# cucapra/pollen

Hardware: AMD Instinct MI355X
Metric: path-steps/sec on `depth` (1M seg / 100M step GFA); bit-exact vs flatgfa CPU (higher is better)
Workload: dtype u32

## Files before the change

pollen_amd/csrc/depth_accum.hip:

```cpp
#include <hip/hip_runtime.h>

#include <cstdlib>

#include "depth_fast_kernels.hpp"
#include "depth_sorted_host.hpp"

namespace fgfa_dev {
namespace {


template <bool UNIQ, int WB>
__device__ __forceinline__ void apply_record(int *D, int *R, uint32_t rec) {
    constexpr uint32_t kW = 1u << WB;
    const uint32_t rel = rec & (kW - 1), end = rel + ((rec >> WB) & ((1u << (kTagShift - WB)) - 1u)) + 1;
    if (UNIQ) {
        const int d = (int)((rec >> 24) & 1u), rv = d - (int)((rec >> 25) & 1u);
        if (d) {
            atomicAdd(&D[rel], 1);
            atomicAdd(&D[end], -1);
        }
        if (rv) {
            atomicAdd(&R[rel], rv);
            atomicAdd(&R[end], -rv);
        }
    } else {
        atomicAdd(&D[rel], 1);
        atomicAdd(&D[end], -1);
    }
}

constexpr uint32_t kPend = 96;
constexpr uint32_t kPendRun = 32;
struct Pending {
    uint32_t *m;
    uint2 *r;
    uint32_t mcnt, rcnt;
    uint32_t moldest;
    int lane;
};

__device__ __forceinline__ uint32_t claim_word(uint32_t *bits, bool act, uint32_t &p, uint32_t e, uint32_t &base) {
    uint32_t rv = 0;
    base = p & ~31u;
    if (act) {
        const uint32_t lo = p & 31u, wl = min(e, p | 31u), width = wl - p + 1u;
        const uint32_t mask = (0xFFFFFFFFu >> (32u - width)) << lo;
        rv = mask & atomicOr(&bits[p >> 5], mask);
        p = wl + 1u;
    }
    return rv;
}
__device__ __forceinline__ void park_rest(Pending &q, bool e, uint32_t val) {
    const unsigned long long mk = __builtin_amdgcn_ballot_w64(e);
    if (e) q.m[q.mcnt + lane_rank(mk)] = val;
    q.mcnt = __builtin_amdgcn_readfirstlane(q.mcnt + (uint32_t)__builtin_popcountll(mk));
}
__device__ __forceinline__ void park_revisit(Pending &q, bool e, uint32_t base, uint32_t rv) {
    const unsigned long long mk = __builtin_amdgcn_ballot_w64(e);
    if (e) q.r[q.rcnt + lane_rank(mk)] = make_uint2(base, rv);
    q.rcnt = __builtin_amdgcn_readfirstlane(q.rcnt + (uint32_t)__builtin_popcountll(mk));
}
template <int WB, int PB = 13>
__device__ __forceinline__ void run_rest(Pending &q, uint32_t *mybits, uint32_t dbg) {
    constexpr uint32_t kNW = (1u << WB) / 32u, kPM = (1u << PB) - 1u;
    const uint32_t n = __builtin_amdgcn_readfirstlane(min(q.mcnt, 64u));
    q.mcnt = __builtin_amdgcn_readfirstlane(q.mcnt - n);
    const bool act = (uint32_t)q.lane < n;
    const uint32_t v = act ? q.m[q.mcnt + q.lane] : 0u;
    asm volatile("" ::: "memory");
    uint32_t p = v & kPM, base;
    const uint32_t e = (v >> PB) & kPM;
    uint32_t rv = claim_word(mybits + (v >> (2 * PB)) * kNW, act, p, e, base);
    if (dbg & kDbgNoRevisit) rv = 0;
    park_rest(q, act && p <= e, (v & ~kPM) | p);
    park_revisit(q, rv != 0u, base, rv);
}
__device__ __forceinline__ void run_revisits(Pending &q, int *R) {
    const uint32_t n = __builtin_amdgcn_readfirstlane(min(q.rcnt, 64u));
    q.rcnt = __builtin_amdgcn_readfirstlane(q.rcnt - n);
    const bool act = (uint32_t)q.lane < n;
    const uint2 v = act ? q.r[q.rcnt + q.lane] : make_uint2(0u, 0u);
    asm volatile("" ::: "memory");
    uint32_t rv = v.y;
    if (rv) {
        const uint32_t low = rv & (0u - rv), sum = rv + low;
        const uint32_t from = (uint32_t)__builtin_ctz(low), to = sum ? (uint32_t)__builtin_ctz(sum) : 32u;
        rv &= sum;
        atomicAdd(&R[v.x + from], 1);
        atomicAdd(&R[v.x + to], -1);
    }
    park_revisit(q, rv != 0u, v.x, rv);
}
template <int WB, int PB = 13>
__device__ __forceinline__ void run_pending(Pending &q, int *R, uint32_t *mybits, uint32_t dbg, uint32_t at_least) {
    while (q.mcnt >= at_least || q.rcnt >= at_least) {
        if (q.rcnt >= at_least) run_revisits(q, R);
        else run_rest<WB, PB>(q, mybits, dbg);
        if (at_least == 1u && q.mcnt == 0u && q.rcnt == 0u) break;
    }
}

struct Claim {
    uint32_t old, mask, p, e, base, slot;
    bool act;
};
template <int WB, bool POINT = false>
__device__ __forceinline__ Claim claim_begin(int *D, Pending &q, uint32_t *mybits, uint32_t slot, uint32_t hfirst, uint32_t rec, bool valid, uint32_t dbg) {
    constexpr uint32_t kW = 1u << WB, kNW = kW / 32u;
    Claim c;
    const uint32_t rel = rec & (kW - 1);
    if (POINT) {
        c.e = rel;
        if (valid) {
            atomicAdd(&D[rel], 1);
            atomicAdd(&D[rel + 1u], -1);
        }
        c.act = valid;
        c.slot = slot;
        c.base = rel & ~31u;
        c.mask = 1u << (rel & 31u);
        c.p = rel + 1u;
        c.old = valid ? atomicOr(&mybits[slot * kNW + (rel >> 5)], c.mask) : 0u;
        return c;
    }
    c.e = rel + ((rec >> WB) & 1023u);
    if (valid && !(dbg & kDbgNoDepth)) {
        atomicAdd(&D[rel], 1);
        atomicAdd(&D[c.e + 1u], -1);
    }
    c.act = valid && !(dbg & kDbgNoClaim);
    c.slot = slot;
    c.base = rel & ~31u;
    const uint32_t lo = rel & 31u, wl = min(c.e, rel | 31u), width = wl - rel + 1u;
    c.mask = (0xFFFFFFFFu >> (32u - width)) << lo;
    c.p = wl + 1u;
    c.old = c.act ? atomicOr(&mybits[slot * kNW + (rel >> 5)], c.mask) : 0u;
    if (q.mcnt == 0u) q.moldest = __builtin_amdgcn_readfirstlane(hfirst);
    return c;
}
template <int WB, bool POINT = false, int PB = 13>
__device__ __forceinline__ void claim_end(int *R, Pending &q, uint32_t *mybits, const Claim &c, uint32_t dbg) {
    uint32_t rv = c.act ? (c.mask & c.old) : 0u;
    if (dbg & kDbgNoRevisit) rv = 0;
    if (POINT) {
        if (rv) {
            atomicAdd(&R[c.e], 1);
            atomicAdd(&R[c.e + 1u], -1);
        }
        return;
    }
    park_rest(q, c.act && c.p <= c.e, c.p | (c.e << PB) | (c.slot << (2 * PB)));
    park_revisit(q, rv != 0u, c.base, rv);
    run_pending<WB, PB>(q, R, mybits, dbg, kPendRun);
}

template <typename T, int N>
__device__ __forceinline__ void block_scan(T *wave_tot, T (&v)[N]) {
    const int tid = threadIdx.x, lane = tid & 63, wave = tid >> 6;
#pragma unroll
    for (int k = 1; k < N; ++k) v[k] += v[k - 1];
    T incl = v[N - 1];
    for (int off = 1; off < 64; off <<= 1) {
        const T t = __shfl_up(incl, off, 64);
        if (lane >= off) incl += t;
    }
    if (lane == 63) wave_tot[wave] = incl;
    __syncthreads();
    T add = incl - v[N - 1];
    for (int k = 0; k < wave; ++k) add += wave_tot[k];
    __syncthreads();
#pragma unroll
    for (int k = 0; k < N; ++k) v[k] += add;
}

template <int N>
__device__ __forceinline__ void store_n(uint32_t *out, uint32_t i0, uint32_t nvalid, const uint32_t (&a)[N]) {
    if (N == 2) {
        if (i0 + 1 < nvalid) *reinterpret_cast<uint2 *>(out + i0) = make_uint2(a[0], a[1]);
        else if (i0 < nvalid) out[i0] = a[0];
        return;
    }
#pragma unroll
    for (int k0 = 0; k0 + 3 < N; k0 += 4) {
        if (i0 + k0 + 3 < nvalid) {
            *reinterpret_cast<uint4 *>(out + i0 + k0) = make_uint4(a[k0], a[k0 + 1], a[k0 + 2], a[k0 + 3]);
        } else {
            for (uint32_t k = 0; k < 4; ++k)
                if (i0 + k0 + k < nvalid) out[i0 + k0 + k] = a[k0 + k];
        }
    }
}

template <int N>
__device__ __forceinline__ void add_n(uint32_t *out, uint32_t i0, uint32_t nvalid, const uint32_t (&a)[N]) {
#pragma unroll
    for (int k = 0; k < N; ++k)
        if (a[k] && i0 + k < nvalid) atomicAdd(out + i0 + k, a[k]);
}

template <bool UNIQ, int kPer>
__device__ __forceinline__ void window_counts(const int *D, const int *R, unsigned long long *wave_tot, uint32_t i0, uint32_t (&d)[kPer], uint32_t (&rv)[kPer]) {
    if (UNIQ) {
        unsigned long long v[kPer];
#pragma unroll
        for (int k = 0; k < kPer; ++k) v[k] = (unsigned long long)(long long)D[i0 + k] + ((unsigned long long)(long long)R[i0 + k] << 32);
        block_scan<unsigned long long, kPer>(wave_tot, v);
#pragma unroll
        for (int k = 0; k < kPer; ++k) {
            d[k] = (uint32_t)v[k];
            rv[k] = (uint32_t)(v[k] >> 32);
        }
    } else {
        int v[kPer];
#pragma unroll
        for (int k = 0; k < kPer; ++k) v[k] = D[i0 + k];
        block_scan<int, kPer>(reinterpret_cast<int *>(wave_tot), v);
#pragma unroll
        for (int k = 0; k < kPer; ++k) d[k] = (uint32_t)v[k];
    }
}
template <bool UNIQ, int kPer>
__device__ __forceinline__ void write_counts(const AccArgs &A, uint32_t w0, uint32_t i0, uint32_t nvalid, bool add, const uint32_t (&d)[kPer], const uint32_t (&u)[kPer]) {
    if (add) {
        add_n<kPer>(A.depth_out + w0, i0, nvalid, d);
        if (UNIQ) add_n<kPer>(A.uniq_out + w0, i0, nvalid, u);
    } else {
        store_n<kPer>(A.depth_out + w0, i0, nvalid, d);
        if (UNIQ) store_n<kPer>(A.uniq_out + w0, i0, nvalid, u);
    }
}

template <bool UNIQ, int WB, int kPerRound = 16>
__device__ __forceinline__ void apply_flat(const AccArgs &A, int *D, int *R, const uint32_t *scnt, const uint32_t *sstart, const uint32_t *wbase) {
    const int lane = threadIdx.x & 63;
    const uint32_t uw = __builtin_amdgcn_readfirstlane(blockIdx.y * kAccWaves + (threadIdx.x >> 6)), nw = A.parts * kAccWaves;
    for (uint32_t s0 = uw; s0 < A.n_slots; s0 += kPerRound * nw) {
        uint4 r[kPerRound];
        uint32_t cnt[kPerRound];
#pragma unroll
        for (int k = 0; k < kPerRound; ++k) {
            const uint32_t s = s0 + k * nw;
            const uint32_t sc = s < A.n_slots ? s : 0u;
            cnt[k] = s < A.n_slots ? scnt[sc] : 0u;
            r[k] = reinterpret_cast<const uint4 *>(wbase + sstart[sc])[(uint32_t)lane < (cnt[k] >> 2) ? lane : 0];
        }
#pragma unroll
        for (int k = 0; k < kPerRound; ++k) {
            if ((uint32_t)lane < (cnt[k] >> 2)) {
                apply_record<UNIQ, WB>(D, R, r[k].x);
                apply_record<UNIQ, WB>(D, R, r[k].y);
                apply_record<UNIQ, WB>(D, R, r[k].z);
                apply_record<UNIQ, WB>(D, R, r[k].w);
            }
        }
#pragma unroll 1
        for (int k = 0; k < kPerRound; ++k) {
            const uint32_t s = s0 + k * nw;
            if (s >= A.n_slots) break;
            const uint32_t c = scnt[s];
            const uint32_t *bk = wbase + sstart[s];
            for (uint32_t i = 64 + lane; i < (c >> 2); i += 64) {
                const uint4 v = reinterpret_cast<const uint4 *>(bk)[i];
                apply_record<UNIQ, WB>(D, R, v.x);
                apply_record<UNIQ, WB>(D, R, v.y);
                apply_record<UNIQ, WB>(D, R, v.z);
                apply_record<UNIQ, WB>(D, R, v.w);
            }
            const uint32_t rest = (c & ~3u) + lane;
            if (rest < c) apply_record<UNIQ, WB>(D, R, bk[rest]);
        }
    }
}

template <int K>
__device__ __forceinline__ void rec_request(const uint32_t *p) {
#ifndef FGFA_REC_POLICY
#define FGFA_REC_POLICY ""
#endif
    if (K == 0) asm volatile("global_load_dword v120, %0, off" FGFA_REC_POLICY ::"v"(p) : "memory", "v120");
    else if (K == 1) asm volatile("global_load_dword v121, %0, off" FGFA_REC_POLICY ::"v"(p) : "memory", "v121");
    else asm volatile("global_load_dword v122, %0, off" FGFA_REC_POLICY ::"v"(p) : "memory", "v122");
}
template <int K>
__device__ __forceinline__ uint32_t rec_take() {
    uint32_t r;
    if (K == 0) asm volatile("s_waitcnt vmcnt(2)\n\tv_mov_b32 %0, v120" : "=v"(r)::"memory");
    else if (K == 1) asm volatile("s_waitcnt vmcnt(2)\n\tv_mov_b32 %0, v121" : "=v"(r)::"memory");
    else asm volatile("s_waitcnt vmcnt(2)\n\tv_mov_b32 %0, v122" : "=v"(r)::"memory");
    return r;
}

template <int WB, bool SHARED, bool POINT, bool BIG>
__device__ __forceinline__ void apply_groups(const AccArgs &A, int *D, int *R, uint32_t *mybits, uint32_t *mark, uint32_t *pend, const uint32_t *wbase, uint32_t win,
                                             uint32_t e0, uint32_t e1, bool have_first = false, uint2 be_first = make_uint2(0u, 0u), uint32_t slf_first = 0u) {
    constexpr uint32_t kNW = (1u << WB) / 32u;
    constexpr uint32_t kSlots = WB <= 12 ? 8u : 4u;
    const int lane = threadIdx.x & 63;
    const uint32_t wave = __builtin_amdgcn_readfirstlane(blockIdx.y * kAccWaves + (threadIdx.x >> 6)), nw = A.parts * kAccWaves;
    const uint32_t nback = (A.has_pre && !SHARED) ? min(__builtin_amdgcn_readfirstlane(*A.work_counter), A.max_back) : 0u;
    const uint32_t nst = e1 - e0;
    const uint32_t nE = nst + (nback > wave ? (nback - wave + nw - 1u) / nw : 0u);
    uint32_t gbase = 0, carryG = 0;
    uint32_t hbase = 0, hdone = 0;
    Pending pq;
    pq.m = pend;
    pq.r = reinterpret_cast<uint2 *>(pend + kPend);
    pq.mcnt = pq.rcnt = pq.moldest = 0;
    pq.lane = lane;
    uint2 be_next = make_uint2(0u, 0u);
    uint32_t slf_next = 0u;
    const auto fetch = [&](uint32_t mb) {
        const uint32_t x = mb + (uint32_t)lane;
        const uint32_t at = x < nst ? e0 + x : A.n_items + wave + nw * (x - nst);
        be_next = x < nE ? A.dir[(size_t)win * A.dstride + at] : make_uint2(0u, 0u);
        slf_next = x < nE ? A.islot[at] : 0u;
    };
    if (have_first) {
        be_next = be_first;
        slf_next = slf_first;
    } else {
        fetch(0);
    }
    for (uint32_t mb = 0; mb < nE; mb += 64u) {
        const uint2 be = be_next;
        const uint32_t slf = slf_next;
        fetch(mb + 64u);
        const uint32_t sl = slf & 0x7FFFFFFFu, first = slf >> 31;
        const uint32_t b = min(be.x, A.cap), en = max(b, min(be.y, A.cap));
        const uint32_t n = en - b;
        const uint32_t incl = wave_scan_incl(n), P = incl - n;
        const uint32_t T = __builtin_amdgcn_readlane(incl, 63);
        const uint32_t G = gbase + wave_scan_incl(first);
        gbase = __builtin_amdgcn_readlane(G, 63);
        const unsigned long long ne = __builtin_amdgcn_ballot_w64(n != 0u);
        const unsigned long long below = ne & ((1ull << lane) - 1ull);
        const int pv = below ? 63 - __builtin_clzll(below) : 0;
        const uint32_t gsh = __shfl(G, pv, 64);
        const uint32_t gprev = below ? gsh : carryG;
        const uint32_t H = hbase + wave_scan_incl((n != 0u && gprev != G) ? 1u : 0u);
        hbase = __builtin_amdgcn_readlane(H, 63);
        if (ne) carryG = __builtin_amdgcn_readlane(G, 63 - __builtin_clzll(ne));
        const uint32_t offH = (sl * A.cap + b) | (H << 24);
        uint32_t cs = 0, lastE = 0;
        uint32_t curEnd = 0;
        uint32_t hseen = hdone;
        struct Chunk {
            const uint32_t *src;
            uint32_t slot;
            uint32_t nv, hl, hf;
        };
        auto prep = [&]() -> Chunk {
            Chunk c;
            const uint32_t q = cs + (uint32_t)lane;
            if (BIG && cs + 64u <= curEnd) {
                const uint32_t oh = __builtin_amdgcn_readlane(offH, lastE), Ps = __builtin_amdgcn_readlane(P, lastE);
                const uint32_t h = oh >> 24;
                c.hf = c.hl = h;
                c.nv = 64u;
                c.src = wbase + (oh & 0xFFFFFFu) + (q - Ps);
                c.slot = h & (kSlots - 1u);
                hseen = h;
                cs += 64u;
                return c;
            }
            const uint32_t relp = P - cs;
            mark[lane] = 0u;
            if (n != 0u && relp < 64u) mark[relp] = (uint32_t)lane + 1u;
            asm volatile("" ::: "memory");
            const uint32_t sel = max(wave_scan_max(mark[lane]), lastE + 1u) - 1u;
            const uint32_t oh = __shfl(offH, (int)sel, 64), Ps = __shfl(P, (int)sel, 64);
            const uint32_t h = oh >> 24;
// ... 626 lines not shown
        const uint32_t at = x < nst ? ge0 + x : A.n_items + vwave + nw * (x - nst);
        if (x < nE) {
            be_first = A.dir[(size_t)win * A.dstride + at];
            slf_first = A.islot[at];
        }
    }
    for (uint32_t sl = tid; sl < A.n_slots; sl += kAccThreads) {
        if ((sl % nw) / kAccWaves != blockIdx.y) {
            sstart[sl] = A.pk ? A.pk[(size_t)win * A.n_slots + sl].x : sl * A.cap;
            continue;
        }
        uint32_t *c = A.counts + (size_t)win * A.n_slots + sl;
        uint32_t v = *c;
        if (!A.keep) *c = 0u;
        uint32_t start = sl * A.cap, room = A.cap;
        if (A.pk) {
            const uint2 e = A.pk[(size_t)win * A.n_slots + sl];
            start = e.x;
            room = e.y;
        } else if (v > (A.cap >> 1)) {
            atomicMax(A.status + 2, v);
            if (A.fullest) atomicMax(A.fullest, v);
        }
        sstart[sl] = start;
        if (TAGGED && UNIQ) {
            const uint32_t c1 = min(v, room);
            v = min(A.has_pre == 1 ? A.counts0[(size_t)win * A.n_slots + sl] : A.has_pre ? v : 0u, c1);
            scnt2[sl] = make_uint2(start + v, (c1 - v) | (A.taken && A.taken[sl] <= (uint32_t)SLOTS ? 0x80000000u : 0u));
        } else if (UNIQ && A.has_pre == 1) {
            v = A.counts0[(size_t)win * A.n_slots + sl];
        }
        scnt[sl] = min(v, room);
    }
    if (tid == 0) grab = kAccWaves;
    if (TAGGED && UNIQ)
        for (uint32_t i = tid; i < A.n_shared * (kW / 32); i += kAccThreads) tag_bits[kAccWaves * (uint32_t)SLOTS * (kW / 32) + i] = 0u;
    const uint32_t nvalid = min(kW, A.n_segs - w0);
    for (uint32_t i = tid; i < (UNIQ ? 2u : 1u) * (kW + 64); i += kAccThreads) cells[i] = 0;
    __syncthreads();
    const uint32_t *wbase = A.pk ? A.buckets : A.buckets + (size_t)win * A.n_slots * A.cap;
    tm.mark(0);
    if (flat) apply_flat<UNIQ, WB, (LOWREG ? 4 : 16)>(A, D, R, scnt, sstart, wbase);
    tm.mark(1);
    if (UNIQ && TAGGED) {
        if (PAIR) apply_tagged<WB, POINT, false, true, (int)kTagSlots, NC>(A, D, R, tag_bits, scnt2, wbase, &grab);
        else if (LOWREG && A.n_shared) apply_tagged<WB, POINT, true, true, SLOTS, NC>(A, D, R, tag_bits, scnt2, wbase, &grab);
        else if (LOWREG) apply_tagged<WB, POINT, false, true, SLOTS, NC>(A, D, R, tag_bits, scnt2, wbase, &grab);
        else if (A.n_shared) apply_tagged<WB, POINT, true, false, SLOTS, NC, OWN>(A, D, R, tag_bits, scnt2, wbase, &grab);
        else apply_tagged<WB, POINT, false, false, SLOTS, NC, OWN>(A, D, R, tag_bits, scnt2, wbase, &grab);
    } else if (UNIQ) {
        apply_groups<WB, false, POINT, BIG>(A, D, R, bits + wave * (kSlots * (kW / 32)), marks + wave * 64, pend + wave * (3 * kPend), wbase, win,
                                ge0, ge1, true, be_first, slf_first);
        for (uint32_t f = A.fat_off[blockIdx.y]; f < A.fat_off[blockIdx.y + 1]; ++f) {
            __syncthreads();
            for (uint32_t i = tid; i < kW / 32; i += kAccThreads) bits[kW / 32 + i] = 0u;
            __syncthreads();
            const uint32_t *wo = A.fat_woff + (size_t)f * (kAccWaves + 1) + wave;
            apply_groups<WB, true, POINT, BIG>(A, D, R, bits, marks + wave * 64, pend + wave * (3 * kPend), wbase, win,
                                   __builtin_amdgcn_readfirstlane(wo[0]), __builtin_amdgcn_readfirstlane(wo[1]));
        }
    }
    tm.mark(2);
    __syncthreads();
    tm.mark(3);
    const uint32_t i0 = kPer * tid;
    uint32_t d[kPer], u[kPer];
    if (UNIQ) {
        uint32_t rv[kPer];
        window_counts<true, kPer>(D, R, wave_tot, i0, d, rv);
#pragma unroll
        for (int k = 0; k < kPer; ++k) u[k] = d[k] - rv[k];
        if (PAIR) {
            __shared__ uint32_t second;
            uint32_t *mine = A.pair_part + ((size_t)win * 2u + blockIdx.y) * (2u * kW);
            const uint32_t *theirs = A.pair_part + ((size_t)win * 2u + (1u - blockIdx.y)) * (2u * kW);
#pragma unroll
            for (int k = 0; k < kPer; ++k) {
                __hip_atomic_store(mine + i0 + k, d[k], __ATOMIC_RELAXED, __HIP_MEMORY_SCOPE_AGENT);
                __hip_atomic_store(mine + kW + i0 + k, rv[k], __ATOMIC_RELAXED, __HIP_MEMORY_SCOPE_AGENT);
            }
            asm volatile("s_waitcnt vmcnt(0)" ::: "memory");
            __syncthreads();
            if (tid == 0) second = __hip_atomic_fetch_add(&A.pair_flag[win], 1u, __ATOMIC_RELAXED, __HIP_MEMORY_SCOPE_AGENT);
            __syncthreads();
            if (second) {
#pragma unroll
                for (int k = 0; k < kPer; ++k) {
                    d[k] += __hip_atomic_load(theirs + i0 + k, __ATOMIC_RELAXED, __HIP_MEMORY_SCOPE_AGENT);
                    rv[k] += __hip_atomic_load(theirs + kW + i0 + k, __ATOMIC_RELAXED, __HIP_MEMORY_SCOPE_AGENT);
                }
#pragma unroll
                for (int k = 0; k < kPer; ++k) u[k] = d[k] - rv[k];
                if (A.accumulate) {
                    add_n<kPer>(A.depth_out + w0, i0, nvalid, d);
                    add_n<kPer>(A.uniq_out + w0, i0, nvalid, u);
                } else {
                    store_n<kPer>(A.depth_out + w0, i0, nvalid, d);
                    store_n<kPer>(A.uniq_out + w0, i0, nvalid, u);
                }
                if (tid == 0) __hip_atomic_store(&A.pair_flag[win], 0u, __ATOMIC_RELAXED, __HIP_MEMORY_SCOPE_AGENT);
            }
        } else {
            write_counts<true, kPer>(A, w0, i0, nvalid, A.parts > 1 || A.accumulate, d, u);
        }
        tm.mark(4);
        tm.finish();
    } else {
        window_counts<false, kPer>(D, R, wave_tot, i0, d, u);
        write_counts<false, kPer>(A, w0, i0, nvalid, !PSUM && (A.parts > 1 || A.accumulate), d, u);
        if (PSUM) {
            unsigned long long l[kPer], w[kPer];
#pragma unroll
            for (int k = 0; k < kPer; ++k) {
                const uint32_t len = i0 + k < nvalid ? A.seg_len[w0 + i0 + k] : 0u;
                l[k] = len;
                w[k] = (unsigned long long)d[k] * len;
            }
            block_scan<unsigned long long, kPer>(wave_tot, l);
            block_scan<unsigned long long, kPer>(wave_tot, w);
#pragma unroll
            for (int k = 0; k < kPer; ++k) {
                LW[i0 + k + 1] = make_ulonglong2(l[k], w[k]);
            }
            if (tid == 0) LW[0] = make_ulonglong2(0ull, 0ull);
            __syncthreads();
            sum_groups<WB>(A, LW, wbase, win, __builtin_amdgcn_readfirstlane(A.wave_off[vwave]), __builtin_amdgcn_readfirstlane(A.wave_off[vwave + 1]));
            for (uint32_t f = A.fat_off[blockIdx.y]; f < A.fat_off[blockIdx.y + 1]; ++f) {
                const uint32_t *wo = A.fat_woff + (size_t)f * (kAccWaves + 1) + wave;
                sum_groups<WB>(A, LW, wbase, win, __builtin_amdgcn_readfirstlane(wo[0]), __builtin_amdgcn_readfirstlane(wo[1]));
            }
        }
    }
}

template <bool UNIQ, int WB, bool PSUM = false, bool POINT = false, bool BIG = false, bool TAGGED = false, int SLOTS = (int)kTagSlots, bool NC = false, bool OWN = false>
__global__ __launch_bounds__(kAccThreads) void k_accum(const AccArgs A) {
    accum_body<UNIQ, WB, PSUM, POINT, BIG, TAGGED, false, SLOTS, false, NC, OWN>(A);
}
#ifdef FGFA_MEASURE
template <int WB, bool POINT>
__global__ __launch_bounds__(kAccThreads) __attribute__((amdgpu_waves_per_eu(8, 8))) void k_accum_pair(const AccArgs A) {
    accum_body<true, WB, false, POINT, false, true, true, (int)kTagSlots, true, true>(A);
}
template <int WB>
__global__ __launch_bounds__(kAccThreads) __attribute__((amdgpu_waves_per_eu(8, 8))) void k_accum_small(const AccArgs A) {
    accum_body<true, WB, false, false, false, true, false, (int)kTagSlots, true, true>(A);
}
#endif

typedef uint32_t sorted_u32x4 __attribute__((ext_vector_type(4)));
template <bool NT>
__device__ __forceinline__ sorted_u32x4 sorted_load4(const sorted_u32x4 *p) { return NT ? __builtin_nontemporal_load(p) : *p; }

template <bool UNIQ, int WB, bool CHECKED>
__device__ __forceinline__ void sweep_group(int *D, int *R, const sorted_u32x4 &r4, uint32_t carry, bool in, int lane) {
    const uint32_t pad = CHECKED && !in ? kSortedPad : 0u;
    const uint32_t rec[kSortedGroup] = {r4.x | pad, r4.y | pad, r4.z | pad, r4.w | pad};
    if (UNIQ) {
        const uint32_t q = (uint32_t)lane >> 4, seed = CHECKED && !in ? 0u : sorted_seed(q, carry);
        SortedLane ln;
        sorted_lane_keys<CHECKED>(rec, q, (uint32_t)WB, seed, ln);
        uint32_t p = sorted_umax(seed, wave_scan_max((uint32_t)__builtin_amdgcn_update_dpp(0u, ln.t, 0x138 , 0xf, 0xf, true)));
#pragma unroll
        for (uint32_t k = 0; k < kSortedGroup; ++k) {
            uint32_t end;
            const bool hit = sorted_record_step<CHECKED>(p, ln.x[k], ln.len[k], end);
            if (!CHECKED || ln.x[k] != 0u) {
                atomicAdd(&D[ln.s[k]], 1);
                atomicAdd(&D[ln.s[k] + ln.len[k] + 1u], -1);
            }
            if (hit) {
                atomicAdd(&R[ln.s[k]], 1);
                atomicAdd(&R[end], -1);
            }
        }
    } else {
        constexpr uint32_t kW = 1u << WB;
#pragma unroll
        for (uint32_t k = 0; k < kSortedGroup; ++k) {
            const uint32_t s = rec[k] & (kW - 1u), e = s + ((rec[k] >> WB) & 1023u) + 1u;
            if (!CHECKED || !(rec[k] & kSortedPad)) {
                atomicAdd(&D[s], 1);
                atomicAdd(&D[e], -1);
            }
        }
    }
}

template <bool UNIQ, int WB, bool NT>
__global__ __launch_bounds__(kAccThreads) __attribute__((amdgpu_waves_per_eu(8, 8))) void k_accum_sorted(const AccArgs A) {
    static_assert(kSortedChunk == 64u && kSortedGroup == 4u, "a lane holds four consecutive records of one chunk: sixteen lanes a chunk");
    constexpr uint32_t kW = 1u << WB;
    constexpr int kPer = kW / kAccThreads;
    __shared__ __attribute__((aligned(16))) int cells[(UNIQ ? 2 : 1) * (kW + 64)];
    __shared__ unsigned long long wave_tot[kAccWaves];
    int *D = cells, *R = cells + (UNIQ ? kW + 64 : 0);
    const int tid = threadIdx.x, lane = tid & 63;
    const uint32_t wave = __builtin_amdgcn_readfirstlane(tid >> 6);
    const uint32_t win = blockIdx.x, w0 = win * kW;
    const uint32_t c0 = __builtin_amdgcn_readfirstlane(A.swin_chunk[win]), c1 = __builtin_amdgcn_readfirstlane(A.swin_chunk[win + 1]);
    const uint32_t ng = (c1 - c0 + kSortedGroup - 1u) / kSortedGroup;
    const sorted_u32x4 *img = reinterpret_cast<const sorted_u32x4 *>(A.srec);
    const uint32_t q = (uint32_t)lane >> 4;
    uint32_t g = wave;
    sorted_u32x4 ra, rb;
    uint32_t ca = 0u, cb = 0u;
    const auto request = [&](sorted_u32x4 &r, uint32_t &cy, uint32_t at) {
        const uint32_t ck = c0 + at * kSortedGroup;
        r = sorted_load4<NT>(img + min(ck * (kSortedChunk / kSortedGroup) + (uint32_t)lane, c1 * (kSortedChunk / kSortedGroup) - 1u));
        if (UNIQ) cy = A.scarry[min(ck + q, c1 - 1u)];
    };
    const auto sweep = [&](const sorted_u32x4 &r, uint32_t cy, uint32_t at) {
        if (at + 1u == ng) sweep_group<UNIQ, WB, true>(D, R, r, cy, c0 + at * kSortedGroup + q < c1, lane);
        else sweep_group<UNIQ, WB, false>(D, R, r, cy, true, lane);
    };
    if (ng) request(ra, ca, g);
    for (uint32_t i = tid; i < (UNIQ ? 2u : 1u) * (kW + 64); i += kAccThreads) cells[i] = 0;
    __syncthreads();
    while (g < ng) {
        request(rb, cb, g + kAccWaves);
        sweep(ra, ca, g);
        g += kAccWaves;
        if (g >= ng) break;
        request(ra, ca, g + kAccWaves);
        sweep(rb, cb, g);
        g += kAccWaves;
    }
    __syncthreads();
    const uint32_t nvalid = min(kW, A.n_segs - w0), i0 = kPer * tid;
    uint32_t d[kPer], u[kPer];
    window_counts<UNIQ, kPer>(D, R, wave_tot, i0, d, u);
    if (UNIQ) {
#pragma unroll
        for (int k = 0; k < kPer; ++k) u[k] = d[k] - u[k];
    }
    write_counts<UNIQ, kPer>(A, w0, i0, nvalid, A.accumulate != 0u, d, u);
}

}

bool accum_kernels_setup() {
    static OncePerDevice once;
    const bool ok = once([] {
        bool good = true;
        const auto set = [&](const void *k, uint32_t bytes) { good = hipFuncSetAttribute(k, hipFuncAttributeMaxDynamicSharedMemorySize, (int)bytes) == hipSuccess && good; };
        set((const void *)k_accum<true, 11, false, false, false, true>, tagged_lds_bytes(11, kMaxShared));
        set((const void *)k_accum<true, 12, false, false, false, true>, tagged_lds_bytes(12, kMaxShared));
        set((const void *)k_accum<true, 12, false, true, false, true>, tagged_lds_bytes(12, kMaxShared));
        set((const void *)k_accum<true, 12, false, false, false, true, 8>, tagged_lds_bytes(12, 64, 8));
        set((const void *)k_accum<true, 13, false, false, false, true>, tagged_lds_bytes(13, 0));
        set((const void *)k_accum<true, 13, false, true, false, true>, tagged_lds_bytes(13, 0));
        set((const void *)k_accum<true, 11, false, false, false, true, (int)kTagSlots, true>, tagged_lds_bytes(11, kMaxShared));
        set((const void *)k_accum<true, 12, false, false, false, true, (int)kTagSlots, true>, tagged_lds_bytes(12, kMaxShared));
        set((const void *)k_accum<true, 12, false, true, false, true, (int)kTagSlots, true>, tagged_lds_bytes(12, kMaxShared));
        set((const void *)k_accum<true, 12, false, false, false, true, 8, true>, tagged_lds_bytes(12, 64, 8));
        set((const void *)k_accum<true, 13, false, false, false, true, (int)kTagSlots, true>, tagged_lds_bytes(13, 0));
        set((const void *)k_accum<true, 13, false, true, false, true, (int)kTagSlots, true>, tagged_lds_bytes(13, 0));
        set((const void *)k_accum<true, 12, false, false, false, true, (int)kTagSlots, false, true>, tagged_lds_bytes(12, kMaxShared));
        set((const void *)k_accum<true, 12, false, false, false, true, 8, false, true>, tagged_lds_bytes(12, 64, 8));
        set((const void *)k_accum<true, 13, false, false, false, true, (int)kTagSlots, false, true>, tagged_lds_bytes(13, 0));
        set((const void *)k_accum<true, 12, false, false, false, true, (int)kTagSlots, true, true>, tagged_lds_bytes(12, kMaxShared));
        set((const void *)k_accum<true, 12, false, false, false, true, 8, true, true>, tagged_lds_bytes(12, 64, 8));
        set((const void *)k_accum<true, 13, false, false, false, true, (int)kTagSlots, true, true>, tagged_lds_bytes(13, 0));
#ifdef FGFA_MEASURE
        set((const void *)k_accum_small<11>, tagged_lds_bytes(11, kMaxShared));
        set((const void *)k_accum_pair<12, false>, tagged_lds_bytes(12, 0));
        set((const void *)k_accum_pair<12, true>, tagged_lds_bytes(12, 0));
#endif
        return good;
    });
    if (!ok) set_error("hipFuncSetAttribute(k_accum): dynamic shared memory");
    return ok;
}

#define FGFA_TAGGED_LAUNCH(GRID, LDS, WB_, POINT_, SLOTS_)                                                                      \
    do {                                                                                                                       \
        if (nc) hipLaunchKernelGGL((k_accum<true, WB_, false, POINT_, false, true, SLOTS_, true>), GRID, dim3(kAccThreads), LDS, stream, aa);  \
        else hipLaunchKernelGGL((k_accum<true, WB_, false, POINT_, false, true, SLOTS_, false>), GRID, dim3(kAccThreads), LDS, stream, aa);    \
    } while (0)
#define FGFA_OWN_LAUNCH(GRID, LDS, WB_, SLOTS_)                                                                                \
    do {                                                                                                                       \
        if (nc) hipLaunchKernelGGL((k_accum<true, WB_, false, false, false, true, SLOTS_, true, true>), GRID, dim3(kAccThreads), LDS, stream, aa);  \
        else hipLaunchKernelGGL((k_accum<true, WB_, false, false, false, true, SLOTS_, false, true>), GRID, dim3(kAccThreads), LDS, stream, aa);    \
    } while (0)
#define FGFA_SORTED_LAUNCH(WB_)                                                                                                  \
    do {                                                                                                                        \
        if (uniq && fp.sorted_nt) hipLaunchKernelGGL((k_accum_sorted<true, WB_, true>), dim3(fp.n_win), dim3(kAccThreads), 0, stream, aa);        \
        else if (uniq) hipLaunchKernelGGL((k_accum_sorted<true, WB_, false>), dim3(fp.n_win), dim3(kAccThreads), 0, stream, aa);                  \
        else if (fp.sorted_nt) hipLaunchKernelGGL((k_accum_sorted<false, WB_, true>), dim3(fp.n_win), dim3(kAccThreads), 0, stream, aa);          \
        else hipLaunchKernelGGL((k_accum_sorted<false, WB_, false>), dim3(fp.n_win), dim3(kAccThreads), 0, stream, aa);                           \
    } while (0)
void launch_accum(const FastPlan &fp, AccArgs &aa, bool uniq, bool tagged, bool psum, hipStream_t stream, bool sorted) {
    if (sorted) {
        if (fp.wb == 11) FGFA_SORTED_LAUNCH(11);
        else if (fp.wb == 12) FGFA_SORTED_LAUNCH(12);
        else FGFA_SORTED_LAUNCH(13);
        return;
    }
    const dim3 agrid(fp.n_win, fp.acc_parts);
    const bool pair = uniq && tagged && fp.acc_pair;
    const bool nc = fp.n_noclaim != 0 || fp.n_flag_chunks != 0;
#ifdef FGFA_MEASURE
    if (pair) {
        aa.parts = 2;
        const uint32_t tl = tagged_lds_bytes(fp.wb, 0);
        const dim3 pgrid(fp.n_win, 2);
        if (fp.dense) hipLaunchKernelGGL((k_accum_pair<12, true>), pgrid, dim3(kAccThreads), tl, stream, aa);
        else hipLaunchKernelGGL((k_accum_pair<12, false>), pgrid, dim3(kAccThreads), tl, stream, aa);
    } else
#else
    (void)pair;
#endif
    if (uniq && tagged) {
        const uint32_t tl = tagged_lds_bytes(fp.wb, fp.n_shared);
        if (fp.dense && fp.wb == 12) FGFA_TAGGED_LAUNCH(agrid, tl, 12, true, (int)kTagSlots);
        else if (fp.dense && fp.wb == 13) FGFA_TAGGED_LAUNCH(agrid, tl, 13, true, (int)kTagSlots);
#ifdef FGFA_MEASURE
        else if (fp.wb == 11 && test_hook("FLATGFA_ACC_SMALL")) hipLaunchKernelGGL((k_accum_small<11>), agrid, dim3(kAccThreads), tl, stream, aa);
#endif
        else if (fp.wb == 11) FGFA_TAGGED_LAUNCH(agrid, tl, 11, false, (int)kTagSlots);
        else if (fp.acc_own && fp.wb == 12 && fp.acc_slots == 8 && fp.n_shared <= 64) FGFA_OWN_LAUNCH(agrid, tagged_lds_bytes(12, fp.n_shared, 8), 12, 8);
        else if (fp.acc_own && fp.wb == 12) FGFA_OWN_LAUNCH(agrid, tl, 12, (int)kTagSlots);
        else if (fp.acc_own && fp.wb == 13) FGFA_OWN_LAUNCH(agrid, tl, 13, (int)kTagSlots);
        else if (fp.wb == 12 && fp.acc_slots == 8 && fp.n_shared <= 64) FGFA_TAGGED_LAUNCH(agrid, tagged_lds_bytes(12, fp.n_shared, 8), 12, false, 8);
        else if (fp.wb == 12) FGFA_TAGGED_LAUNCH(agrid, tl, 12, false, (int)kTagSlots);
        else FGFA_TAGGED_LAUNCH(agrid, tl, 13, false, (int)kTagSlots);
    } else if (uniq) {
        const bool big = fp.big_groups;
        if (fp.dense && fp.wb == 12 && big) hipLaunchKernelGGL((k_accum<true, 12, false, true, true>), agrid, dim3(kAccThreads), 0, stream, aa);
        else if (fp.dense && fp.wb == 12) hipLaunchKernelGGL((k_accum<true, 12, false, true, false>), agrid, dim3(kAccThreads), 0, stream, aa);
        else if (fp.dense && fp.wb == 13) hipLaunchKernelGGL((k_accum<true, 13, false, true, true>), agrid, dim3(kAccThreads), 0, stream, aa);
        else if (fp.wb == 12 && big) hipLaunchKernelGGL((k_accum<true, 12, false, false, true>), agrid, dim3(kAccThreads), 0, stream, aa);
        else if (fp.wb == 13 && big) hipLaunchKernelGGL((k_accum<true, 13, false, false, true>), agrid, dim3(kAccThreads), 0, stream, aa);
        else if (fp.wb == 11) hipLaunchKernelGGL((k_accum<true, 11>), agrid, dim3(kAccThreads), 0, stream, aa);
        else if (fp.wb == 12) hipLaunchKernelGGL((k_accum<true, 12>), agrid, dim3(kAccThreads), 0, stream, aa);
        else hipLaunchKernelGGL((k_accum<true, 13>), agrid, dim3(kAccThreads), 0, stream, aa);
    } else {
        if (fp.wb == 11) hipLaunchKernelGGL((k_accum<false, 11>), agrid, dim3(kAccThreads), 0, stream, aa);
        else if (fp.wb == 12 && psum) hipLaunchKernelGGL((k_accum<false, 12, true>), agrid, dim3(kAccThreads), 0, stream, aa);
        else if (fp.wb == 12) hipLaunchKernelGGL((k_accum<false, 12>), agrid, dim3(kAccThreads), 0, stream, aa);
        else hipLaunchKernelGGL((k_accum<false, 13>), agrid, dim3(kAccThreads), 0, stream, aa);
    }
}
#undef FGFA_TAGGED_LAUNCH
#undef FGFA_OWN_LAUNCH
#undef FGFA_SORTED_LAUNCH

void launch_path_reduce(const FastPlan &fp, unsigned long long *len_out, unsigned long long *weighted_out, hipStream_t stream) {
    hipLaunchKernelGGL(k_path_reduce, dim3((fp.n_items + 3) / 4), dim3(256), 0, stream, reinterpret_cast<const uint4 *>(fp.items), fp.elist, fp.n_items,
                       fp.n_win, fp.dstride, reinterpret_cast<const ulonglong2 *>(fp.psum_part), len_out, weighted_out);
}

}
```

pollen_amd/csrc/depth_call_host.hpp:

```cpp
#pragma once
#include <algorithm>
#include <cstdint>

#include "depth_fast.hpp"

namespace fgfa_dev {

struct CallHooks {
    bool scan_always = false;
    const char *scan_time = nullptr;
    bool no_plain = false;
    bool acc_time = false;
    const char *acc_skip = nullptr;
};
struct CallWants {
    bool uniq = false;
    bool psum = false, psum_clear = false;
    bool count_only = false;
};
struct GraphFacts {
    uint32_t n_segs;
    bool has_seg_len;
};
enum class Zeroes { nobody, k_scan, memset };
struct CallShape {
    const char *refusal = nullptr;
    bool has_pre = false;
    bool scan_skip = false;
    uint32_t grid = 0;
    uint32_t grid_tiny = 0, grid_short = 0, grid_medium = 0;
    bool tagged = false, ranged = false, big = false, cflags = false;
    bool from_image = false;
    bool kept = false;
    bool sorted = false;
    uint32_t has_pre2 = 0;
    uint32_t max_back = 0;
    Zeroes outputs = Zeroes::nobody, sums = Zeroes::nobody;
    bool scans() const { return grid && !kept; }
};

constexpr int kModeDense = -1, kModeRefused = -2;
struct ScanMode {
    int mode;
    bool tagged;
};
inline ScanMode scan_mode(const FastPlan &fp, const CallShape &s) {
    if (fp.dense) return {kModeDense, false};
#ifdef FGFA_MEASURE
    if (fp.dbg) return {kModeDbg, false};
#endif
    const bool flags = s.cflags && s.tagged && !s.ranged;
    if (flags && fp.packed) return {kModePackedFlags, true};
    if (flags && !s.big) return {kModePlainFlags, true};
    if (fp.packed) return {s.ranged ? kModePackedRanged : kModePacked, true};
    if (s.big && !s.tagged) return {kModeRefused, false};
    if (s.big) return {s.ranged ? kModeRangedBig : kModeBig, true};
    if (s.ranged) return {kModeRanged, s.tagged};
    return {s.tagged && fp.narrow_emit ? kModePlainNarrow : kModePlain, s.tagged};
}

inline uint32_t wave_list_grid(uint32_t n, uint32_t per_wg, uint32_t n_slots) { return std::min<uint32_t>((n + per_wg - 1) / per_wg, n_slots); }

inline CallShape decide_call(const FastPlan &fp, const GraphFacts &g, const CallWants &w, const CallHooks &hooks, bool records_use) {
    CallShape s;
    if (w.psum && (w.uniq || fp.wb != 12 || !g.has_seg_len || !fp.psum_part || fp.n_range != g.n_segs)) {
        s.refusal = "fast_seg_depth: path sums ride on seg_depth with 4096-segment windows only";
        return s;
    }
    const bool tagged = fp.tagged && !w.psum;
    if (fp.packed && !tagged) {
        s.refusal = "fast_seg_depth: a plan with packed buckets runs tagged calls only";
        return s;
    }
    s.tagged = tagged;
    s.has_pre = fp.n_short || fp.n_medium || fp.n_tiny;
    s.scan_skip = s.has_pre && fp.n_items == 0 && fp.exact_short && !fp.dbg && !hooks.scan_always;
    s.grid = s.scan_skip ? 0u : s.has_pre ? fp.n_slots : std::min<uint32_t>(fp.n_items, fp.n_slots);
    s.has_pre2 = s.scan_skip ? 2u : s.has_pre ? 1u : 0u;
    s.max_back = s.scan_skip ? 0u : fp.max_back;
    s.ranged = fp.seg_base != 0 || fp.n_range != g.n_segs;
    const uint32_t stride = fp.n_slots * fp.cap;
    s.big = ((uint64_t)fp.n_win + 1) * stride >= (1ull << 30);
    s.cflags = tagged && fp.cflags;
    s.from_image = s.grid && tagged && fp.run_ent && fp.run_item_ent && !w.count_only && !fp.dense && !fp.packed && !s.ranged && !s.cflags && !s.has_pre && !fp.dbg;
    s.kept = s.from_image && records_use && fp.counts_kept;
    s.sorted = s.kept && fp.sorted_rec && fp.sorted_carry && fp.sorted_win_chunk && fp.acc_parts == 1 && fp.wb >= 11 && fp.wb <= 13;
    if (s.scans() && !s.from_image && scan_mode(fp, s).mode == kModeRefused) {
        CallShape no;
        no.refusal = "fast_seg_depth: a bucket array this large needs a tagged call";
        return no;
    }
    if (fp.n_tiny) s.grid_tiny = wave_list_grid(fp.n_tiny, kWaves, fp.n_slots);
    if (fp.n_short) s.grid_short = wave_list_grid(fp.n_short, kShortWaves, fp.n_slots);
    if (fp.n_medium) s.grid_medium = wave_list_grid(fp.n_medium, kMediumPaired ? kMediumWaves / 2 : kMediumWaves, fp.n_slots);
    const Zeroes who = s.scans() ? Zeroes::k_scan : Zeroes::memset;
    if (fp.acc_parts > 1 && !fp.accumulate && !w.count_only) s.outputs = who;
    if (w.psum && w.psum_clear) s.sums = s.grid ? Zeroes::k_scan : Zeroes::memset;
    return s;
}

enum class StatusVerdict {
    fine,
    bounds, stale, internal, several_calls,
    redo_grown,
    redo_atomic,
    unresolved,
};
struct StatusAction {
    StatusVerdict verdict;
    bool grow_ahead;
};
inline StatusAction status_verdict(const uint32_t st3[3], uint32_t calls, int attempt, bool last_fast, bool has_last_call) {
    const uint32_t st = st3[0], over = kStOverflow | kStBackOverflow;
    StatusAction a{StatusVerdict::fine, st3[2] != 0 && !(st & over)};
    if (st & kStBounds) a.verdict = StatusVerdict::bounds;
    else if (st & kStStale) a.verdict = StatusVerdict::stale;
    else if (st & kStInternal) a.verdict = StatusVerdict::internal;
    else if (!(st & over)) a.verdict = StatusVerdict::fine;
    else if (attempt == 0 && calls > 1) a.verdict = StatusVerdict::several_calls;
    else if (!last_fast || !has_last_call || attempt > 8) a.verdict = StatusVerdict::unresolved;
    else a.verdict = (st & kStBackOverflow) ? StatusVerdict::redo_atomic : StatusVerdict::redo_grown;
    return a;
}

}
```

pollen_amd/csrc/depth_device.hip:

```cpp
#include <hip/hip_runtime.h>

#include <algorithm>
#include <atomic>
#include <chrono>
#include <cstdio>
#include <cstdlib>
#include <cstring>
#include <mutex>
#include <string>
#include <vector>

#include "../../include/flatgfa.h"
#include "depth_call_host.hpp"
#include "depth_fast.hpp"
#include "depth_sorted_host.hpp"
#include "temp_arena.hpp"
#include "host_copy.hpp"
#include "device_common.hpp"
#include "prof.hpp"

namespace fgfa_dev {

thread_local std::string g_last_error;
void set_error(const std::string &s) { g_last_error = s; }
// ... 91 lines not shown
            if (seg >= n_segs) {
                *status = 1u;
                continue;
            }
            if (win == 0) atomicAdd(&depth[seg], 1u);
            const uint32_t rel = seg - lo;
            if (rel < nbits) {
                const uint32_t bit = 1u << (rel & 31u);
                const uint32_t old = atomicOr(&seen[rel >> 5], bit);
                if (!(old & bit)) atomicAdd(&uniq[seg], 1u);
            }
        }
        __syncthreads();
    }
}

constexpr int kSumThreads = 256;

__global__ __launch_bounds__(256) void k_zero_outputs(uint32_t *__restrict__ a, uint32_t *__restrict__ b, uint32_t n) {
    for (uint32_t i = blockIdx.x * 256u + threadIdx.x; i < n; i += gridDim.x * 256u) {
        a[i] = 0u;
        if (b) b[i] = 0u;
    }
}

__global__ __launch_bounds__(256) void k_pack_len_depth(const uint32_t *__restrict__ seg_len,
                                                        const uint32_t *__restrict__ depth, uint32_t n_segs,
                                                        uint2 *__restrict__ tab) {
    for (uint32_t s = blockIdx.x * blockDim.x + threadIdx.x; s < n_segs; s += gridDim.x * blockDim.x)
        tab[s] = make_uint2(seg_len[s], depth[s]);
}

__global__ __launch_bounds__(kSumThreads) void k_path_sums(const uint32_t *__restrict__ steps,
                                                            const uint32_t *__restrict__ path_begin,
                                                            const uint32_t *__restrict__ path_end, uint32_t n_paths,
                                                            uint32_t n_segs, const uint2 *__restrict__ tab,
                                                            const uint32_t *__restrict__ path_ids, uint32_t n_ids,
                                                            uint32_t split, uint32_t by_path,
                                                            unsigned long long *__restrict__ length_out,
                                                            unsigned long long *__restrict__ weighted_out,
                                                            uint32_t *__restrict__ status) {
    __shared__ unsigned long long red[2][kSumThreads / 64];
    const uint64_t total = (uint64_t)n_ids * split;
    for (uint64_t job = blockIdx.x; job < total; job += gridDim.x) {
        const uint32_t k = (uint32_t)(job / split), part = (uint32_t)(job % split);
        const uint32_t p = path_ids[k];
        unsigned long long len = 0, wsum = 0;
        if (p < n_paths) {
            const uint64_t b = path_begin[p], e = path_end[p];
            const uint64_t n = e - b;
            const uint64_t lo = b + n * part / split, hi = b + n * (part + 1) / split;
            constexpr int kBatch = 8;
            bool bad = false;
            uint64_t i = lo + threadIdx.x;
            for (; i + (uint64_t)(kBatch - 1) * kSumThreads < hi; i += (uint64_t)kBatch * kSumThreads) {
                uint32_t seg[kBatch];
                uint2 ld[kBatch];
#pragma unroll
                for (int k = 0; k < kBatch; ++k) seg[k] = steps[i + (uint64_t)k * kSumThreads] >> 1;
#pragma unroll
                for (int k = 0; k < kBatch; ++k) {
                    bad |= seg[k] >= n_segs;
                    ld[k] = tab[seg[k] < n_segs ? seg[k] : 0u];
                }
#pragma unroll
                for (int k = 0; k < kBatch; ++k) {
                    const bool ok = seg[k] < n_segs;
                    len += ok ? (unsigned long long)ld[k].x : 0ull;
                    wsum += ok ? (unsigned long long)ld[k].y * ld[k].x : 0ull;
                }
            }
            for (; i < hi; i += kSumThreads) {
                const uint32_t seg = steps[i] >> 1;
                const bool ok = seg < n_segs;
                const uint2 ld = tab[ok ? seg : 0u];
                bad |= !ok;
                len += ok ? (unsigned long long)ld.x : 0ull;
                wsum += ok ? (unsigned long long)ld.y * ld.x : 0ull;
            }
            if (bad) *status = 1u;
        } else if (threadIdx.x == 0 && part == 0) {
            *status = 1u;
        }
        for (int off = 32; off > 0; off >>= 1) {
            len += __shfl_down(len, off, 64);
            wsum += __shfl_down(wsum, off, 64);
        }
        const int lane = threadIdx.x & 63, wave = threadIdx.x >> 6;
        if (lane == 0) {
            red[0][wave] = len;
            red[1][wave] = wsum;
        }
        __syncthreads();
        if (threadIdx.x == 0) {
            unsigned long long a = 0, c = 0;
            for (int w = 0; w < kSumThreads / 64; ++w) {
                a += red[0][w];
                c += red[1][w];
            }
            const uint32_t at = by_path ? p : k;
            if (a) atomicAdd(&length_out[at], a);
            if (c) atomicAdd(&weighted_out[at], c);
        }
        __syncthreads();
    }
}

}


using namespace fgfa_dev;

struct flatgfa_dev_plan {
    flatgfa_dev_graph_t g;
    int device = 0;
    int n_cus = 256;
    WorkItem *items = nullptr;
    uint32_t n_items = 0;
    uint32_t *status = nullptr;
    uint32_t n_windows = 1;
    FastPlan fast;
    uint32_t *overlap_bits = nullptr;
    uint32_t *overlap_qbits = nullptr;
    size_t overlap_qbytes = 0;
    bool overlap_qall = false;
    uint2 *len_depth = nullptr;
    uint32_t *last_depth = nullptr, *last_uniq = nullptr;
    uint64_t *last_len = nullptr, *last_weighted = nullptr;
    bool last_fast = false;
    uint32_t calls_since_status = 0;
    uint32_t *all_ids = nullptr;
    int64_t cache_claim = 0;
    bool cache_claim_shared = false;
    std::vector<uint32_t> hb, he;
    uint32_t scan_workgroups = 0;
    hipStream_t side = nullptr;
    std::vector<MarksJob> marks;
    bool marks_to_start = false;
    bool check_facts = false;
    struct RunShare *run = nullptr;
    void *run_item_ent = nullptr;
    void *run_room = nullptr;
    hipEvent_t run_items_done = nullptr;
    int run_state = 0;
    const char *run_off = "";
    bool run_show = false;
    int run_hook = -1;
    bool records_kept = false;
    bool keep_records = true;
    struct SortedShare *sorted = nullptr;
    int sorted_state = 0;
    const char *sorted_off = "";
    int sorted_hook = -1;
};

static int plan_fast_call(flatgfa_dev_plan_t *pl, uint32_t *depth_out, uint32_t *uniq_out, hipStream_t stream, const PathSums *ps = nullptr) {
    RecordsUse ru;
    ru.use = pl->keep_records && pl->records_kept;
    pl->records_kept = false;
    const int rc = fast_seg_depth(pl->fast, pl->g, depth_out, uniq_out, pl->status, stream, ps, &ru);
    pl->records_kept = rc == FLATGFA_OK && pl->keep_records && ru.from_image;
    return rc;
}
static bool plan_grow(flatgfa_dev_plan_t *pl, bool ahead_of_need = false) {
    pl->records_kept = false;
    return fast_plan_grow(&pl->fast, ahead_of_need);
}

static std::mutex g_cache_mu;
static int64_t g_cache_claimed[64] = {};
struct CacheShare {
    int device;
    const uint32_t *steps;
    int64_t bytes;
    int users;
};
static std::vector<CacheShare> g_cache_shares;

extern "C" int flatgfa_dev_path_overlaps_impl(const flatgfa_dev_graph_t *g, int n_cus, uint32_t **coarse_cache,
                                              uint32_t **qbits_cache, size_t *qbits_bytes, bool *qbits_all, const uint32_t *query_ids, uint32_t n_q, uint8_t *touch_out,
                                              uint32_t *status, hipStream_t stream);

static int atomic_seg_depth(flatgfa_dev_plan_t *pl, uint32_t *depth_out, uint32_t *uniq_out, hipStream_t stream);

static flatgfa_dev_plan_t *plan_create_impl(const flatgfa_dev_graph_t *g, const uint32_t *hb, const uint32_t *he, uint32_t scan_workgroups,
                                            uint32_t *first_depth = nullptr, uint32_t *first_uniq = nullptr, int *first_status = nullptr);
extern "C" flatgfa_dev_plan_t *flatgfa_dev_plan_create(const flatgfa_dev_graph_t *g, const uint32_t *hb,
                                                        const uint32_t *he) {
    return plan_create_impl(g, hb, he, 0u);
}
extern "C" flatgfa_dev_plan_t *flatgfa_dev_plan_create_first(const flatgfa_dev_graph_t *g, const uint32_t *hb, const uint32_t *he,
                                                              uint32_t *depth_out, uint32_t *uniq_out, int *first_status) {
    if (g && g->n_segs && !depth_out) { set_error("dev_plan_create_first: NULL depth_out"); return nullptr; }
    return plan_create_impl(g, hb, he, 0u, depth_out, uniq_out, first_status);
}

static int device_cus(int device) {
    static std::mutex mu;
    static int cus[64] = {};
    std::lock_guard<std::mutex> lk(mu);
    if (device >= 0 && device < 64 && cus[device]) return cus[device];
    hipDeviceProp_t prop;
    int n = 256;
    if (hipGetDeviceProperties(&prop, device) == hipSuccess && prop.multiProcessorCount > 0) n = prop.multiProcessorCount;
    else (void)hipGetLastError();
    if (device >= 0 && device < 64) cus[device] = n;
    return n;
}
namespace fgfa_dev {
int device_cu_count(int device) { return device_cus(device); }
void plan_tick(const char *what) {
    static const char *const mode = getenv("FLATGFA_TIMING");
    if (!mode) return;
    static const bool drain = std::string(mode) != "host";
    static thread_local std::chrono::steady_clock::time_point last = std::chrono::steady_clock::now();
    if (what) {
        const auto before = std::chrono::steady_clock::now();
        if (drain) (void)hipDeviceSynchronize();
        const auto now = std::chrono::steady_clock::now();
        fprintf(stderr, "plan: %-52s %8.3f ms (+ %.3f ms for the device to drain)\n", what, std::chrono::duration<double, std::milli>(before - last).count(),
                std::chrono::duration<double, std::milli>(now - before).count());
    }
    last = std::chrono::steady_clock::now();
}
}

static void release_cache_claim(flatgfa_dev_plan_t *pl) {
    if (!pl->cache_claim) return;
    std::lock_guard<std::mutex> lk(g_cache_mu);
    bool last = true;
    if (pl->cache_claim_shared) {
        for (size_t i = 0; i < g_cache_shares.size(); ++i) {
            CacheShare &c = g_cache_shares[i];
            if (c.device != pl->device || c.steps != pl->g.steps) continue;
            last = --c.users == 0;
            if (last) g_cache_shares.erase(g_cache_shares.begin() + (long)i);
            break;
        }
    }
    if (last && pl->device >= 0 && pl->device < 64) g_cache_claimed[pl->device] -= pl->cache_claim;
    pl->cache_claim = 0;
    pl->cache_claim_shared = false;
}

static hipStream_t side_stream(flatgfa_dev_plan_t *pl) {
    if (pl->side) return pl->side;
    static std::mutex mu;
    static hipStream_t pool[64] = {};
    std::lock_guard<std::mutex> lk(mu);
    hipStream_t &slot = pool[pl->device >= 0 && pl->device < 64 ? pl->device : 0];
    if (!slot) {
        int least = 0, greatest = 0;
        if (hipDeviceGetStreamPriorityRange(&least, &greatest) != hipSuccess) { (void)hipGetLastError(); least = 0; }
        if (hipStreamCreateWithPriority(&slot, hipStreamNonBlocking, least) != hipSuccess) { (void)hipGetLastError(); slot = nullptr; return nullptr; }
    }
    pl->side = slot;
    return slot;
}

struct RunShare {
    int device;
    const uint32_t *steps;
    uint64_t n_steps;
    RunImage *img;
    hipStream_t side;
    int users;
    bool listed;
    bool any_ratio;
    std::vector<struct SortedShare *> sorted;
};
struct SortedShare {
    fgfa_dev::SortedImage *img;
    flatgfa_dev_plan_t *builder;
    uint32_t wb, n_win, n_range, n_segs;
    std::vector<uint32_t> hb, he;
    int users;
};
static std::mutex g_run_mu;
static std::vector<RunShare *> g_run_shares;
static std::atomic<int> g_side_pending[64];
constexpr uint64_t kRunImageReserve = 1ull << 30;
static void side_work_wait(int device) {
    if (device < 0 || device >= 64 || !g_side_pending[device].load(std::memory_order_acquire)) return;
    std::lock_guard<std::mutex> lk(g_run_mu);
    g_side_pending[device].store(0, std::memory_order_release);
    hipStream_t side = nullptr;
    for (RunShare *sh : g_run_shares) {
        if (sh->device != device) continue;
        side = sh->side;
        (void)run_image_poll(sh->img, sh->side, true, kRunImageReserve, sh->any_ratio);
    }
    if (side) (void)hipStreamSynchronize(side);
}
static void side_work_enqueued(int device) {
    if (device >= 0 && device < 64) g_side_pending[device].store(1, std::memory_order_release);
}
constexpr bool kRunImageDefault = true;

static void sorted_release(flatgfa_dev_plan_t *pl) {
    pl->fast.sorted_rec = pl->fast.sorted_carry = pl->fast.sorted_win_chunk = nullptr;
    if (SortedShare *ss = pl->sorted) {
        std::lock_guard<std::mutex> lk(g_run_mu);
        if (ss->builder == pl) {
            (void)sorted_image_poll(ss->img, pl->fast, pl->side, true, kRunImageReserve, pl->sorted_hook == 1);
            ss->builder = nullptr;
        }
// ... 1 lines not shown
            if (pl->run) {
                auto &list = pl->run->sorted;
                list.erase(std::remove(list.begin(), list.end(), ss), list.end());
            }
            sorted_image_free(ss->img, pl->side);
            delete ss;
        }
        pl->sorted = nullptr;
    }
    pl->sorted_state = 0;
    pl->sorted_off = "";
}

static void run_release(flatgfa_dev_plan_t *pl, bool steps_changed) {
    sorted_release(pl);
    if (pl->run_items_done) {
        (void)hipEventSynchronize(pl->run_items_done);
        (void)hipEventDestroy(pl->run_items_done);
        pl->run_items_done = nullptr;
    }
    if (pl->run_item_ent) (void)hipFree(pl->run_item_ent);
    if (pl->run_room) (void)hipFree(pl->run_room);
    pl->run_item_ent = pl->run_room = nullptr;
    pl->fast.run_ent = pl->fast.run_item_ent = nullptr;
    if (RunShare *sh = pl->run) {
        std::lock_guard<std::mutex> lk(g_run_mu);
        sh->users -= 1;
        if (sh->listed && (steps_changed || sh->users == 0)) {
            g_run_shares.erase(std::find(g_run_shares.begin(), g_run_shares.end(), sh));
            sh->listed = false;
        }
        if (sh->users == 0) {
            run_image_free(sh->img, sh->side);
            delete sh;
        }
        pl->run = nullptr;
    }
    pl->run_state = 0;
    pl->run_off = "";
}

static const char *run_image_refused(flatgfa_dev_plan_t *pl) {
    const FastPlan &f = pl->fast;
    const flatgfa_dev_graph_t &g = pl->g;
    const bool hook = pl->run_hook >= 0, forced = pl->run_hook == 1;
    const bool by_size = (uint64_t)g.n_steps * 4 >= (64ull << 20);
    pl->run_show = by_size || hook;
    if (pl->run_hook == 0) return "hook";
    if (!forced && !kRunImageDefault) return "default";
    if (!forced && !by_size) return "small";
    if (!f.eligible) return "atomic";
    if (f.n_items && ((uint64_t)f.n_items + std::min(f.n_items, f.n_slots) - 1) / std::min(f.n_items, f.n_slots) > f.tag_limit) return "items";
    if (!f.tagged) return "untagged";
    if (f.n_more || f.n_groups > 1 || f.seg_base || f.n_range != g.n_segs) return "ranges";
    if (f.packed) return "packed";
    if (f.dense) return "dense";
    if (f.n_short || f.n_medium || f.n_tiny) return "short_paths";
    if (!f.n_items) return "no_items";
    if (f.cflags) return "marks";
    if (pl->check_facts) return "check_no_claim";
    if (f.dbg) return "debug";
    if (f.wb < 11 || f.wb > 13) return "windows";
    std::vector<std::pair<uint32_t, uint32_t>> spans;
    for (size_t p = 0; p < pl->hb.size(); ++p)
        if (pl->he[p] > pl->hb[p]) spans.push_back({pl->hb[p], pl->he[p]});
    std::sort(spans.begin(), spans.end());
    for (size_t i = 1; i < spans.size(); ++i)
        if (spans[i].first < spans[i - 1].second) return "overlap";
    return nullptr;
}

static void sorted_poll(flatgfa_dev_plan_t *pl, bool wait);
static void run_poll(flatgfa_dev_plan_t *pl, bool wait, bool may_start, hipStream_t behind = nullptr) {
    if (pl->run_state < 0 || (pl->run_state == 3 && (pl->sorted_state == 3 || pl->sorted_state < 0))) return;
    if (pl->run_state == 0 && !may_start) return;
    DeviceGuard guard;
    if (guard.dev < 0 || !guard.switch_to(pl->device)) { (void)hipGetLastError(); return; }
    if (pl->run_state == 3) { sorted_poll(pl, wait); return; }
    const auto give_up = [&](const char *why) {
        run_release(pl, false);
        pl->run_state = -1;
        pl->run_off = why;
    };
    if (pl->run_state == 0) {
        if (const char *why = run_image_refused(pl)) { give_up(why); return; }
        hipStream_t side = side_stream(pl);
        if (!side) { give_up("error"); return; }
        std::lock_guard<std::mutex> lk(g_run_mu);
        if (behind) {
            hipEvent_t after = nullptr;
            if (hipEventCreateWithFlags(&after, hipEventDisableTiming) == hipSuccess) {
                if (hipEventRecord(after, behind) == hipSuccess) (void)hipStreamWaitEvent(side, after, 0);
                (void)hipEventDestroy(after);
            }
            (void)hipGetLastError();
        }
        for (RunShare *sh : g_run_shares)
            if (sh->device == pl->device && sh->steps == pl->g.steps && sh->n_steps == pl->g.n_steps) pl->run = sh;
        if (!pl->run) {
            pl->run = new RunShare{pl->device, pl->g.steps, pl->g.n_steps, run_image_start(pl->g, side), side, 0, true, pl->run_hook == 1, {}};
            g_run_shares.push_back(pl->run);
            side_work_enqueued(pl->device);
        }
        pl->run->users += 1;
        pl->run_state = 1;
    }
    if (pl->run_state == 1) {
        int r;
        {
            std::lock_guard<std::mutex> lk(g_run_mu);
            r = run_image_poll(pl->run->img, pl->run->side, wait, kRunImageReserve, pl->run->any_ratio);
            side_work_enqueued(pl->device);
            if (r > 0 && !run_items_start(pl->fast, pl->run->img, pl->run->side, &pl->run_item_ent, &pl->run_room, &pl->run_items_done)) r = -2;
        }
        if (r == 0) return;
        if (r < 0) { give_up(r == -2 ? "error" : run_image_why(pl->run->img)); return; }
        pl->run_state = 2;
    }
    if (pl->run_state == 2) {
        const hipError_t e = wait ? hipEventSynchronize(pl->run_items_done) : hipEventQuery(pl->run_items_done);
        if (e == hipErrorNotReady) { (void)hipGetLastError(); return; }
        if (e != hipSuccess) { (void)hipGetLastError(); give_up("error"); return; }
        const uint32_t room = run_room_needed(pl->fast, pl->run_room);
        (void)hipFree(pl->run_room);
        pl->run_room = nullptr;
        if (room == ~0u) { give_up("error"); return; }
        if (room > pl->fast.cap) {
            (void)hipDeviceSynchronize();
            for (int k = 0; k < 3 && room > pl->fast.cap && pl->fast.eligible && !pl->fast.cap_forced; ++k)
                if (!plan_grow(pl)) { pl->fast.eligible = true; break; }
            if (room > pl->fast.cap) { give_up("room"); return; }
        }
        const int64_t traffic = (int64_t)run_image_bytes(pl->run->img) + 8ll * (int64_t)pl->g.n_segs + 8ll * (int64_t)pl->fast.est_records;
        const char *mall = getenv("FLATGFA_MALL_MB");
        const bool nt = traffic > (244ll << 20) || (mall && strtoull(mall, nullptr, 10) == 0);
        pl->records_kept = false;
        if (pl->keep_records && !pl->fast.counts_kept) {
            const size_t bytes = (size_t)pl->fast.n_win * pl->fast.n_slots * 4;
            if (hipMalloc(&pl->fast.counts_kept, bytes) != hipSuccess) {
                (void)hipGetLastError();
                pl->fast.counts_kept = nullptr;
            } else if (hipMemset(pl->fast.counts_kept, 0, bytes) != hipSuccess || hipStreamSynchronize(nullptr) != hipSuccess) {
                (void)hipGetLastError();
                (void)hipFree(pl->fast.counts_kept);
                pl->fast.counts_kept = nullptr;
            }
        }
        run_image_install(&pl->fast, pl->run->img, pl->run_item_ent, nt);
        pl->run_state = 3;
        sorted_poll(pl, wait);
    }
}

static void sorted_poll(flatgfa_dev_plan_t *pl, bool wait) {
    if (pl->sorted_state == 3 || pl->sorted_state < 0 || pl->run_state != 3) return;
    const auto give_up = [&](const char *why) {
        sorted_release(pl);
        pl->sorted_state = -1;
        pl->sorted_off = why;
    };
    const FastPlan &f = pl->fast;
    hipStream_t side = pl->run->side;
    if (pl->sorted_state == 0) {
        if (const char *why = sorted_refused(pl->sorted_hook, f.acc_parts, f.n_groups, f.n_more, f.wb, pl->keep_records && f.counts_kept)) { give_up(why); return; }
        std::lock_guard<std::mutex> lk(g_run_mu);
        for (SortedShare *ss : pl->run->sorted)
            if (ss->wb == f.wb && ss->n_win == f.n_win && ss->n_range == f.n_range && ss->n_segs == pl->g.n_segs && ss->hb == pl->hb && ss->he == pl->he) pl->sorted = ss;
        if (!pl->sorted) {
            pl->sorted = new SortedShare{sorted_image_start(f, pl->g.n_paths, side), pl, f.wb, f.n_win, f.n_range, pl->g.n_segs, pl->hb, pl->he, 0};
            pl->run->sorted.push_back(pl->sorted);
            side_work_enqueued(pl->device);
        }
        pl->sorted->users += 1;
        pl->sorted_state = 1;
    }
    int r;
    const char *why = "";
    {
        std::lock_guard<std::mutex> lk(g_run_mu);
        SortedShare *ss = pl->sorted;
        const int before = sorted_image_phase(ss->img);
        r = sorted_image_poll(ss->img, ss->builder ? ss->builder->fast : f, side, wait, kRunImageReserve, pl->sorted_hook == 1);
        if (before == 1 && sorted_image_phase(ss->img) == 2) side_work_enqueued(pl->device);
        if (r != 0) ss->builder = nullptr;
        if (r < 0) why = sorted_image_why(ss->img);
    }
    if (r == 0) return;
    if (r < 0) { give_up(why); return; }
    const int64_t traffic = (int64_t)sorted_image_bytes(pl->sorted->img) + 8ll * (int64_t)pl->g.n_segs;
    const char *mall = getenv("FLATGFA_MALL_MB");
    const bool nt = traffic > (244ll << 20) || (mall && strtoull(mall, nullptr, 10) == 0);
    sorted_image_install(&pl->fast, pl->sorted->img, nt);
    pl->sorted_state = 3;
}

static void marks_start(flatgfa_dev_plan_t *pl);
static void marks_jobs_poll(flatgfa_dev_plan_t *pl, bool wait);
static void marks_poll(flatgfa_dev_plan_t *pl, bool wait, bool before_a_call = false) {
    if (before_a_call) {
        side_work_wait(pl->device);
        wait = wait || pl->run_state > 0;
    }
    marks_jobs_poll(pl, wait && !before_a_call);
    if (pl->marks.empty() && !pl->marks_to_start) run_poll(pl, wait, !before_a_call);
}
static void run_start_behind(flatgfa_dev_plan_t *pl, hipStream_t stream) {
    if (pl->run_state == 0 && pl->marks.empty() && !pl->marks_to_start) run_poll(pl, false, true, stream);
}
static void marks_jobs_poll(flatgfa_dev_plan_t *pl, bool wait) {
    if (pl->marks_to_start) {
        pl->marks_to_start = false;
        marks_start(pl);
    }
    if (pl->marks.empty()) return;
    bool pending = false;
    for (size_t k = 0; k < pl->marks.size(); ++k) {
        MarksJob &job = pl->marks[k];
        if (!job.active) continue;
        if (!wait && !fast_marks_ready(job)) { pending = true; continue; }
        FastPlan *fp = k == 0 ? &pl->fast : (k - 1 < pl->fast.n_more ? &pl->fast.more[k - 1] : nullptr);
        if (fp) fast_marks_finish(fp, &job);
    }
    if (!pending) pl->marks.clear();
}
static void marks_start(flatgfa_dev_plan_t *pl) {
    if (!pl->fast.eligible) return;
    if (!any_range(pl->fast, [](const FastPlan &q) { return q.marks_wanted; })) return;
    DeviceGuard guard;
    if (guard.dev < 0 || !guard.switch_to(pl->device)) { (void)hipGetLastError(); return; }
    if (!side_stream(pl)) return;
    pl->marks.assign(1 + pl->fast.n_more, MarksJob());
    for (size_t k = 0; k < pl->marks.size(); ++k) {
        const FastPlan &fp = k == 0 ? pl->fast : pl->fast.more[k - 1];
        if (fp.eligible && fp.marks_wanted) (void)fast_marks_start(fp, pl->g, pl->hb.data(), pl->side, &pl->marks[k]);
    }
}


static void claim_cache(flatgfa_dev_plan_t *pl) {
    const flatgfa_dev_graph_t *g = &pl->g;
    if (!(pl->fast.eligible && g->n_steps && pl->fast.n_items)) return;
    uint64_t records = 0;
    for_each_range(pl->fast, [&](const FastPlan &q) { records += q.est_records; });
    int64_t budget = (244ll << 20) - 8ll * (int64_t)g->n_segs - 8ll * (int64_t)records;
    budget = std::min<int64_t>(budget, 160ll << 20);
    if (const char *f = getenv("FLATGFA_MALL_MB")) budget = (int64_t)strtoull(f, nullptr, 10) << 20;
    budget = std::min<int64_t>(budget, (int64_t)g->n_steps * 4);
    {
        std::lock_guard<std::mutex> lk(g_cache_mu);
        const bool pinned = getenv("FLATGFA_MALL_MB") != nullptr;
        CacheShare *share = nullptr;
        for (CacheShare &c : g_cache_shares)
            if (c.device == pl->device && c.steps == g->steps) share = &c;
        if (pl->device < 0 || pl->device >= 64) {
            budget = 0;
        } else if (share && !pinned) {
            budget = std::min<int64_t>(share->bytes, (int64_t)g->n_steps * 4);
            share->users += 1;
            pl->cache_claim = share->bytes;
            pl->cache_claim_shared = true;
        } else {
            if (!pinned) {
                budget = std::min<int64_t>(budget, (160ll << 20) - g_cache_claimed[pl->device]);
                if (budget < (32ll << 20) || (int64_t)g->n_steps * 4 < (64ll << 20)) budget = 0;
            }
            budget = std::max<int64_t>(budget, 0);
            g_cache_claimed[pl->device] += budget;
            pl->cache_claim = budget;
            if (budget && !pinned) {
                g_cache_shares.push_back(CacheShare{pl->device, g->steps, budget, 1});
                pl->cache_claim_shared = true;
            }
        }
    }
    for_each_range(pl->fast, [&](FastPlan &q) { q.mall_steps = (uint64_t)budget / 4; });
}

struct TrialOutputs {
    uint32_t *depth, *uniq;
};
static int bucketed_query(flatgfa_dev_plan_t *pl, const TrialOutputs &out) {
    return plan_fast_call(pl, out.depth, out.uniq, nullptr);
}

static int remake_with_packed_buckets(flatgfa_dev_plan_t *pl) {
    if (!pl->fast.eligible || getenv("FLATGFA_PACKED")) return 0;
    uint64_t even_bytes = 0;
    for_each_range(pl->fast, [&](const FastPlan &q) { if (!q.packed) even_bytes += ((uint64_t)q.n_win + 1) * q.n_slots * q.cap * 4; });
    if (even_bytes <= (2ull << 30)) return 0;
    if (!all_ranges(pl->fast, [](const FastPlan &q) { return q.can_pack; })) return 0;
    FastPlan again;
    if (!fast_plan_create(pl->g, pl->hb.data(), pl->he.data(), &again, pl->scan_workgroups, true)) return -1;
    if (!(again.eligible && all_ranges(again, [](const FastPlan &q) { return q.packed; }))) {
        fast_plan_destroy(&again);
        return 0;
    }
    for_each_range(again, [&](FastPlan &q) { q.mall_steps = pl->fast.mall_steps; });
    plan_tick("the plan made again with packed buckets");
    fast_plan_destroy(&pl->fast);
    pl->fast = again;
    plan_tick("the even plan's scratch freed");
    return 1;
}

static bool size_buckets(flatgfa_dev_plan_t *pl, const TrialOutputs &out, uint32_t *first_st, bool *complete) {
    *complete = false;
    for (int layout = 0; layout < 2; ++layout) {
        for (int attempt = 0; attempt < 10 && pl->fast.eligible; ++attempt) {
            uint32_t st = 0;
            if (bucketed_query(pl, out) != FLATGFA_OK || hipMemcpy(&st, pl->status, 4, hipMemcpyDeviceToHost) != hipSuccess ||
                hipMemset(pl->status, 0, 4) != hipSuccess)
                return false;
            *first_st |= st & 1u;
            *complete = !(st & (4u | 16u));
            if (!(st & 4u)) break;
            (void)plan_grow(pl);
        }
        plan_tick("sizing query");
        {
            uint32_t fullest = 0;
            if (hipMemcpy(&fullest, pl->status + 2, 4, hipMemcpyDeviceToHost) == hipSuccess && fullest && pl->fast.eligible) (void)plan_grow(pl, true);
            (void)hipMemset(pl->status, 0, 12);
        }
        plan_tick("headroom");
        if (layout != 0) break;
        const int again = remake_with_packed_buckets(pl);
        if (again < 0) return false;
        if (!again) break;
    }
    return true;
}

struct Trial {
    bool ok = false;
    float best[2] = {1e30f, 1e30f};
};
struct TrialEvents {
    hipEvent_t e0 = nullptr, e1 = nullptr;
    bool ok;
    TrialEvents() { ok = hipEventCreate(&e0) == hipSuccess && hipEventCreate(&e1) == hipSuccess; }
    ~TrialEvents() {
        if (e0) (void)hipEventDestroy(e0);
        if (e1) (void)hipEventDestroy(e1);
    }
};
// ... 324 lines not shown
static int path_depth_all_enqueue(flatgfa_dev_plan_t *pl, uint32_t *depth_out, uint64_t *length_out, uint64_t *weighted_out,
                                  hipStream_t stream, bool use_fast) {
    const flatgfa_dev_graph_t &g = pl->g;
    use_fast = use_fast && pl->fast.eligible;
    if (use_fast && fast_plan_want_path_sums(&pl->fast)) {
        const PathSums ps{length_out, weighted_out, true};
        int rc = plan_fast_call(pl, depth_out, nullptr, stream, &ps);
        if (rc) return rc;
        if (pl->fast.n_other) rc = path_sums_launch(pl, pl->fast.other_ids, pl->fast.n_other, depth_out, length_out, weighted_out, 1u, stream);
        return rc;
    }
    {
        ProfScope ps("memset_path_sums", stream);
        FGFA_HIP_OR(hipMemsetAsync(length_out, 0, (size_t)g.n_paths * 8, stream), return FLATGFA_ERR_HIP);
        FGFA_HIP_OR(hipMemsetAsync(weighted_out, 0, (size_t)g.n_paths * 8, stream), return FLATGFA_ERR_HIP);
    }
    int rc = use_fast ? plan_fast_call(pl, depth_out, nullptr, stream)
                      : atomic_seg_depth(pl, depth_out, nullptr, stream);
    if (rc) return rc;
    if (!pl->all_ids) {
        std::vector<uint32_t> ids(g.n_paths);
        for (uint32_t i = 0; i < g.n_paths; ++i) ids[i] = i;
        FGFA_HIP_OR(hipMalloc(&pl->all_ids, (size_t)g.n_paths * 4), return FLATGFA_ERR_HIP);
        FGFA_HIP_OR(fgfa_dev::staged_copy(pl->all_ids, ids.data(), (size_t)g.n_paths * 4, hipMemcpyHostToDevice, nullptr), return FLATGFA_ERR_HIP);
    }
    return path_sums_launch(pl, pl->all_ids, g.n_paths, depth_out, length_out, weighted_out, 1u, stream);
}

extern "C" int flatgfa_dev_path_depth_all(flatgfa_dev_plan_t *pl, uint32_t *depth_out, uint64_t *length_out,
                                          uint64_t *weighted_out, void *stream_) {
    if (!pl || (pl->g.n_segs && !depth_out) || (pl->g.n_paths && (!length_out || !weighted_out))) {
        set_error("dev_path_depth_all: NULL argument");
        return FLATGFA_ERR_ARG;
    }
    const flatgfa_dev_graph_t &g = pl->g;
    if (g.n_paths == 0) return g.n_segs ? flatgfa_dev_seg_depth(pl, depth_out, nullptr, stream_) : FLATGFA_OK;
    if (!g.seg_len && g.n_segs) { set_error("dev_path_depth_all: graph image has no seg_len array"); return FLATGFA_ERR_ARG; }
    if (g.n_segs == 0) {
        FGFA_HIP_OR(hipMemsetAsync(length_out, 0, (size_t)g.n_paths * 8, (hipStream_t)stream_), return FLATGFA_ERR_HIP);
        FGFA_HIP_OR(hipMemsetAsync(weighted_out, 0, (size_t)g.n_paths * 8, (hipStream_t)stream_), return FLATGFA_ERR_HIP);
        return FLATGFA_OK;
    }
    if (const int rc = begin_depth_call(pl, depth_out, nullptr, length_out, weighted_out, (hipStream_t)stream_)) return rc;
    return path_depth_all_enqueue(pl, depth_out, length_out, weighted_out, (hipStream_t)stream_, true);
}

extern "C" int flatgfa_dev_path_overlaps(flatgfa_dev_plan_t *pl, const uint32_t *query_ids, uint32_t n_q,
                                         uint8_t *touch_out, void *stream_) {
    if (!pl || (n_q && (!query_ids || !touch_out))) { set_error("dev_path_overlaps: NULL argument"); return FLATGFA_ERR_ARG; }
    return flatgfa_dev_path_overlaps_impl(&pl->g, pl->n_cus, &pl->overlap_bits, &pl->overlap_qbits, &pl->overlap_qbytes, &pl->overlap_qall,
                                          query_ids, n_q, touch_out, pl->status,
                                          (hipStream_t)stream_);
}

static int redo_last_call(flatgfa_dev_plan_t *pl, bool atomic, hipStream_t stream) {
    const bool grown = !atomic && plan_grow(pl);
    if (atomic) pl->fast.eligible = false;
    if (!grown) pl->last_fast = false;
    if (pl->last_len) return path_depth_all_enqueue(pl, pl->last_depth, pl->last_len, pl->last_weighted, stream, grown);
    if (grown) return plan_fast_call(pl, pl->last_depth, pl->last_uniq, stream);
    return atomic_seg_depth(pl, pl->last_depth, pl->last_uniq, stream);
}

extern "C" int flatgfa_dev_status(flatgfa_dev_plan_t *pl, void *stream_) {
    if (!pl) return FLATGFA_ERR_ARG;
    hipStream_t stream = (hipStream_t)stream_;
    for (int attempt = 0;; ++attempt) {
        uint32_t st3[3] = {0, 0, 0};
        FGFA_HIP_OR(hipMemcpyAsync(st3, pl->status, 12, hipMemcpyDeviceToHost, stream), return FLATGFA_ERR_HIP);
        FGFA_HIP_OR(hipStreamSynchronize(stream), return FLATGFA_ERR_HIP);
        const uint32_t st = st3[0];
        if (st3[0] || st3[2]) pl->records_kept = false;
        const uint32_t n_calls = pl->calls_since_status;
        if (attempt == 0) {
            pl->calls_since_status = 0;
            marks_poll(pl, false);
        }
        const StatusAction act = status_verdict(st3, n_calls, attempt, pl->last_fast, pl->last_depth != nullptr);
        if (st3[2]) {
            FGFA_HIP_OR(hipMemsetAsync(pl->status + 2, 0, 4, stream), return FLATGFA_ERR_HIP);
            if (act.grow_ahead && pl->fast.eligible) (void)plan_grow(pl, true);
        }
        if (st) FGFA_HIP_OR(hipMemsetAsync(pl->status, 0, 4, stream), return FLATGFA_ERR_HIP);
        switch (act.verdict) {
        case StatusVerdict::fine: return FLATGFA_OK;
        case StatusVerdict::bounds:
            set_error("a step refers to a segment id (or a query to a path id) that is out of range");
            return FLATGFA_ERR_BOUNDS;
        case StatusVerdict::stale:
            set_error("the step values changed behind the plan (a path it found strictly monotone no longer is, a no-claim mark or a reversed copy no longer holds): "
                      "call flatgfa_dev_plan_steps_changed, or make the plan again");
            return FLATGFA_ERR_STALE_PLAN;
        case StatusVerdict::internal: {
            char what[512] = "";
            (void)flatgfa_dev_plan_describe(pl, what, (int)sizeof what);
            set_error("node depth: internal error (the records of pass 1 were not in the order pass 2 relies on); status words " + std::to_string(st3[0]) + " " +
                      std::to_string(st3[1]) + " " + std::to_string(st3[2]) + ", " + std::to_string(n_calls) + " call(s) since the last status; plan: " + what);
            return FLATGFA_ERR_HIP;
        }
        case StatusVerdict::several_calls:
            set_error("node depth: a call ran out of scratch room (the steps changed behind the plan?) and " + std::to_string(n_calls) +
                      " calls were enqueued since the last flatgfa_dev_status: call it after every call to have such a call completed (status words " + std::to_string(st3[0]) + " " + std::to_string(st3[2]) + ")");
            return FLATGFA_ERR_HIP;
        case StatusVerdict::unresolved:
            set_error("node depth: scratch overflow could not be resolved");
            return FLATGFA_ERR_HIP;
        case StatusVerdict::redo_grown:
        case StatusVerdict::redo_atomic:
            if (const int rc = redo_last_call(pl, act.verdict == StatusVerdict::redo_atomic, stream)) return rc;
        }
    }
}

extern "C" int flatgfa_dev_plan_describe(flatgfa_dev_plan_t *pl, char *out, int cap) {
    if (!pl || !out || cap <= 0) return 0;
    marks_poll(pl, true);
    const FastPlan &f = pl->fast;
    std::string s;
    if (!f.eligible) {
        s = "path=atomic (k_depth_scan / k_depth_uniq_path)";
    } else {
        const CallShape shape = decide_call(f, {pl->g.n_segs, pl->g.seg_len != nullptr}, CallWants(), CallHooks(), false);
        const bool two_chunks = scan_mode(f, shape).mode == kModePlainNarrow && !f.n_more;
        s = "path=bucketed pass1=" + std::string(shape.scan_skip ? "" : f.dense ? "k_scan_dense+" : "k_scan+") + (f.n_short ? "k_scan_short+" : "") + (f.n_medium ? "k_scan_medium+" : "") + (f.n_tiny ? "k_scan_tiny+" : "");
        s.pop_back();
        s += std::string("") +
            " pass2=" + (f.tagged ? (f.n_shared ? "tagged(shared bitsets)" : f.acc_pair ? "tagged(two workgroups per window)" : "tagged") : (f.big_groups ? "directory(one-item shortcut)" : "directory")) +
            " windows=" + std::to_string(f.n_win) + "x" + std::to_string(1u << f.wb) + " ranges=" + std::to_string((f.n_more + 1) / f.n_groups) +
            (f.n_groups > 1 ? " path_groups=" + std::to_string(f.n_groups) : std::string()) +
            (two_chunks ? " emit=two_chunks" : "") +
            " scan_workgroups=" + std::to_string(f.n_slots) + " workgroups_per_window=" + std::to_string(f.acc_parts) + " items=" + std::to_string(f.n_items) + (f.acc_own ? " bitset_owners=tracked" : "") + " no_claim_items=" + std::to_string(f.n_noclaim) + (f.n_flag_chunks ? " no_claim_chunks=" + std::to_string(f.n_flag_chunks) : std::string()) + " no_claim_paths=" + std::to_string(f.short_mono_n + f.medium_mono_n + f.tiny_mono_n) + " split_paths=" + std::to_string(f.n_shared) +
            " short_paths=" + std::to_string(f.n_short) + " medium_paths=" + std::to_string(f.n_medium) + " tiny_paths=" + std::to_string(f.n_tiny) +
            " steps=" + std::to_string(f.class_steps[0]) + "/" + std::to_string(f.class_steps[1]) + "/" + std::to_string(f.class_steps[2]) + "/" + std::to_string(f.class_steps[3]) +
            " bucket_cap=" + std::to_string(f.cap);
        const auto records_of = [](const FastPlan &q) { return q.packed ? q.bucket_records : ((uint64_t)q.n_win + 1) * q.n_slots * q.cap; };
        uint64_t recs = 0;
        for_each_range(f, [&](const FastPlan &q) { recs += records_of(q); });
        const bool packed = any_range(f, [](const FastPlan &q) { return q.packed; });
        s += std::string(" buckets=") + (packed ? "packed" : "even") + " scratch_mb=" + std::to_string((recs * 4 + (1u << 20) - 1) >> 20) +
             " cache_resident_mb=" + std::to_string((f.mall_steps * 4) >> 20);
        if (pl->run_show) {
            if (pl->run_state == 3) {
                std::lock_guard<std::mutex> lk(g_run_mu);
                s += " run_image=" + std::to_string((run_image_bytes(pl->run->img) + (1u << 20) - 1) >> 20) + " run_image_steps=" + std::to_string(pl->run->n_steps) +
                     " run_image_plans=" + std::to_string(pl->run->users) + " run_image_reads=" + (f.run_nt ? "nt" : "plain");
                const auto mb = [](uint64_t bytes) { return std::to_string((bytes + (1u << 20) - 1) >> 20); };
                if (pl->sorted_state == 3 && f.sorted_rec) {
                    s += " sorted_image=" + mb(sorted_image_bytes(pl->sorted->img)) + " sorted_image_build=" + mb(sorted_image_transient(pl->sorted->img)) +
                         " sorted_image_plans=" + std::to_string(pl->sorted->users) + " sorted_chunk=" + std::to_string(kSortedChunk) + " pass2=sorted";
                } else if (pl->sorted_hook != 0) {
                    s += std::string(" pass2=walk(") + (pl->sorted_state < 0 ? pl->sorted_off : "pending") + ")";
                }
                s += std::string(" records=") + (pl->keep_records && f.counts_kept ? "kept" : "rewritten");
            } else {
                s += std::string(" run_image=off(") + (pl->run_state < 0 ? pl->run_off : "pending") + ")";
            }
        }
    }
    const int n = (int)std::min<size_t>(s.size(), (size_t)cap - 1);
    memcpy(out, s.data(), (size_t)n);
    out[n] = 0;
    return n;
}

extern "C" void flatgfa_dev_profile_enable(int on) {
    std::lock_guard<std::mutex> lk(g_prof_mu);
    g_prof_on = on != 0;
}

extern "C" int flatgfa_dev_profile_read(const char **names, float *ms, int cap) {
    std::lock_guard<std::mutex> lk(g_prof_mu);
    int n = 0;
    std::vector<std::pair<int, hipEvent_t>> done;
    for (auto &r : g_prof) {
        (void)hipEventSynchronize(r.b);
        float t = 0.f;
        (void)hipEventElapsedTime(&t, r.a, r.b);
        if (n < cap) {
            names[n] = r.name;
            ms[n] = t;
            ++n;
        }
        done.push_back({r.device, r.a});
        done.push_back({r.device, r.b});
    }
    g_prof.clear();
    for (const auto &de : done) {
        if ((size_t)de.first >= g_event_pool.size()) g_event_pool.resize((size_t)de.first + 1);
        std::vector<hipEvent_t> &pool = g_event_pool[(size_t)de.first];
        if (pool.size() < 256) pool.push_back(de.second);
        else (void)hipEventDestroy(de.second);
    }
    return n;
}

__global__ __launch_bounds__(1024) void k_nothing(uint32_t *sink) {
    extern __shared__ uint32_t lds_nothing[];
    if (sink && threadIdx.x == 4096) sink[0] = lds_nothing[0];
}

namespace fgfa_dev {
void warm_launch(void *stream) { hipLaunchKernelGGL(k_nothing, dim3(1), dim3(64), 0, (hipStream_t)stream, (uint32_t *)nullptr); }
}

extern "C" float flatgfa_dev_profile_overhead_ms(int n_workgroups, int lds_bytes, int reps, void *stream_) {
    hipStream_t stream = (hipStream_t)stream_;
    if (n_workgroups <= 0 || reps <= 0 || lds_bytes < 0 || lds_bytes > 160 * 1024) return -1.f;
    if (hipFuncSetAttribute((const void *)k_nothing, hipFuncAttributeMaxDynamicSharedMemorySize, 160 * 1024) != hipSuccess) return -1.f;
    hipEvent_t a = nullptr, b = nullptr;
    if (hipEventCreateWithFlags(&a, hipEventDisableSystemFence) != hipSuccess || hipEventCreateWithFlags(&b, hipEventDisableSystemFence) != hipSuccess) return -1.f;
    std::vector<float> ts;
    for (int r = 0; r < reps + 2; ++r) {
        (void)hipEventRecord(a, stream);
        hipLaunchKernelGGL(k_nothing, dim3(n_workgroups), dim3(1024), (size_t)lds_bytes, stream, (uint32_t *)nullptr);
        (void)hipEventRecord(b, stream);
        float t = 0.f;
        if (hipEventSynchronize(b) != hipSuccess || hipEventElapsedTime(&t, a, b) != hipSuccess) { ts.clear(); break; }
        if (r >= 2) ts.push_back(t);
    }
    (void)hipEventDestroy(a);
    (void)hipEventDestroy(b);
    if (ts.empty()) return -1.f;
    std::sort(ts.begin(), ts.end());
    return ts[ts.size() / 2];
}

struct flatgfa_dev_pipeline {
    int device = 0;
    std::vector<flatgfa_dev_plan_t *> plans;
    std::vector<hipStream_t> streams;
    std::vector<hipEvent_t> joined;
    hipEvent_t after = nullptr;
    uint64_t n_calls = 0;
};

extern "C" void flatgfa_dev_pipeline_destroy(flatgfa_dev_pipeline_t *p) {
    if (!p) return;
    for (size_t k = 0; k < p->streams.size(); ++k)
        if (p->streams[k]) (void)hipStreamSynchronize(p->streams[k]);
    for (flatgfa_dev_plan_t *pl : p->plans) flatgfa_dev_plan_destroy(pl);
    for (hipEvent_t e : p->joined)
        if (e) (void)hipEventDestroy(e);
    if (p->after) (void)hipEventDestroy(p->after);
    for (hipStream_t st : p->streams)
        if (st) (void)hipStreamDestroy(st);
    delete p;
}

extern "C" flatgfa_dev_pipeline_t *flatgfa_dev_pipeline_create(const flatgfa_dev_graph_t *g, const uint32_t *hb, const uint32_t *he, int calls_in_flight) {
    if (!g || calls_in_flight < 1 || calls_in_flight > 8) { set_error("dev_pipeline_create: bad argument (1 .. 8 calls in flight)"); return nullptr; }
    auto *p = new flatgfa_dev_pipeline();
    FGFA_HIP_OR(hipGetDevice(&p->device), { delete p; return nullptr; });
    for (int k = 0; k < calls_in_flight; ++k) {
        hipStream_t st = nullptr;
        hipEvent_t ev = nullptr;
        if (hipStreamCreateWithFlags(&st, hipStreamNonBlocking) != hipSuccess || hipEventCreateWithFlags(&ev, hipEventDisableTiming) != hipSuccess) {
            set_error("dev_pipeline_create: cannot create a stream");
            if (st) (void)hipStreamDestroy(st);
            flatgfa_dev_pipeline_destroy(p);
            return nullptr;
        }
        p->streams.push_back(st);
        p->joined.push_back(ev);
        const int n_cus = device_cus(p->device);
        const uint32_t wgs = calls_in_flight < 2 ? 0u : (uint32_t)(calls_in_flight >= 3 && g->n_steps <= (1ull << 28) ? n_cus / 2 : n_cus * 11 / 16);
        flatgfa_dev_plan_t *pl = plan_create_impl(g, hb, he, wgs);
        if (!pl) { flatgfa_dev_pipeline_destroy(p); return nullptr; }
        p->plans.push_back(pl);
    }
    if (hipEventCreateWithFlags(&p->after, hipEventDisableTiming) != hipSuccess) { set_error("dev_pipeline_create: cannot create an event"); flatgfa_dev_pipeline_destroy(p); return nullptr; }
    return p;
}

extern "C" int flatgfa_dev_pipeline_seg_depth(flatgfa_dev_pipeline_t *p, uint32_t *depth_out, uint32_t *uniq_out, void *after_stream) {
    if (!p || p->plans.empty()) { set_error("dev_pipeline_seg_depth: NULL pipeline"); return FLATGFA_ERR_ARG; }
    const size_t lane = (size_t)(p->n_calls % p->plans.size());
    if (after_stream != (void *)-1) {
        FGFA_HIP_OR(hipEventRecord(p->after, (hipStream_t)after_stream), return FLATGFA_ERR_HIP);
        FGFA_HIP_OR(hipStreamWaitEvent(p->streams[lane], p->after, 0), return FLATGFA_ERR_HIP);
    }
    p->n_calls += 1;
    return flatgfa_dev_seg_depth(p->plans[lane], depth_out, uniq_out, p->streams[lane]);
}

extern "C" int flatgfa_dev_pipeline_path_depth_all(flatgfa_dev_pipeline_t *p, uint32_t *depth_out, uint64_t *length_out, uint64_t *weighted_out,
                                                    void *after_stream) {
    if (!p || p->plans.empty()) { set_error("dev_pipeline_path_depth_all: NULL pipeline"); return FLATGFA_ERR_ARG; }
    const size_t lane = (size_t)(p->n_calls % p->plans.size());
    if (after_stream != (void *)-1) {
        FGFA_HIP_OR(hipEventRecord(p->after, (hipStream_t)after_stream), return FLATGFA_ERR_HIP);
        FGFA_HIP_OR(hipStreamWaitEvent(p->streams[lane], p->after, 0), return FLATGFA_ERR_HIP);
    }
    p->n_calls += 1;
    return flatgfa_dev_path_depth_all(p->plans[lane], depth_out, length_out, weighted_out, p->streams[lane]);
}

extern "C" int flatgfa_dev_pipeline_join(flatgfa_dev_pipeline_t *p, void *stream) {
    if (!p) { set_error("dev_pipeline_join: NULL pipeline"); return FLATGFA_ERR_ARG; }
    for (size_t k = 0; k < p->streams.size(); ++k) {
        FGFA_HIP_OR(hipEventRecord(p->joined[k], p->streams[k]), return FLATGFA_ERR_HIP);
        FGFA_HIP_OR(hipStreamWaitEvent((hipStream_t)stream, p->joined[k], 0), return FLATGFA_ERR_HIP);
    }
    return FLATGFA_OK;
}

extern "C" int flatgfa_dev_pipeline_status(flatgfa_dev_pipeline_t *p) {
    if (!p) { set_error("dev_pipeline_status: NULL pipeline"); return FLATGFA_ERR_ARG; }
    int rc = FLATGFA_OK;
    for (size_t k = 0; k < p->plans.size(); ++k) {
        const int r = flatgfa_dev_status(p->plans[k], p->streams[k]);
        if (r != FLATGFA_OK && rc == FLATGFA_OK) rc = r;
    }
    return rc;
}

extern "C" int flatgfa_dev_pipeline_steps_changed(flatgfa_dev_pipeline_t *p) {
    if (!p) { set_error("dev_pipeline_steps_changed: NULL pipeline"); return FLATGFA_ERR_ARG; }
    int rc = FLATGFA_OK;
    for (size_t k = 0; k < p->plans.size(); ++k) {
        const int r = flatgfa_dev_plan_steps_changed(p->plans[k], p->streams[k]);
        if (r != FLATGFA_OK && rc == FLATGFA_OK) rc = r;
    }
    return rc;
}

extern "C" int flatgfa_dev_pipeline_describe(flatgfa_dev_pipeline_t *p, char *out, int cap) {
    if (!p || p->plans.empty() || !out || cap <= 0) return 0;
    std::string s = "calls_in_flight=" + std::to_string(p->plans.size()) + " ";
    char buf[768] = "";
    for (size_t k = p->plans.size(); k-- > 0;) (void)flatgfa_dev_plan_describe(p->plans[k], buf, (int)sizeof buf);
    s += buf;
    const int n = (int)std::min<size_t>(s.size(), (size_t)cap - 1);
    memcpy(out, s.data(), (size_t)n);
    out[n] = 0;
    return n;
}

extern "C" int flatgfa_device_count(void) {
    int n = 0;
    if (hipGetDeviceCount(&n) != hipSuccess) return 0;
    return n;
}
```

pollen_amd/csrc/depth_fast.hip:

```cpp
#include <hip/hip_runtime.h>

#include <algorithm>
#include <cstdlib>
#include <cstring>
#include <cstdio>
#include <mutex>
#include <numeric>
#include <string>
#include <vector>

#include "depth_fast_kernels.hpp"
#include "depth_plan_host.hpp"
#include "depth_call_diag.hpp"
#include "device_scan.hpp"
#include "temp_arena.hpp"
#include "host_copy.hpp"
#include "prof.hpp"

namespace fgfa_dev {
namespace {

struct RunCounts {
    uint32_t run = 0, down = 0, asc = 0, desc = 0, up = 0, dn = 0;
};
// ... 1176 lines not shown
    sa.n_segs = fp.n_range;
    sa.seg_base = fp.seg_base;
    sa.n_total = g.n_segs;
    sa.ranged = s.ranged ? 1u : 0u;
    sa.n_win = fp.n_win;
    sa.n_slots = fp.n_slots;
    sa.wb = fp.wb;
    sa.nwp = fp.nwp;
    sa.has_pre = s.has_pre ? 1u : 0u;
    sa.max_back = s.max_back;
    sa.work_counter = fp.work_counter;
    sa.counts = fp.counts;
    sa.counts0 = fp.counts0;
    sa.buckets = fp.buckets;
    sa.dir = reinterpret_cast<uint2 *>(fp.dir);
    sa.islot = fp.islot;
    sa.perm = fp.perm;
    sa.dstride = fp.dstride;
    sa.cap = fp.cap;
    sa.stride = fp.n_slots * fp.cap;
    sa.sink = fp.n_win * sa.stride;
    sa.big = s.big ? 1u : 0u;
    sa.status = status;
    sa.dbg = fp.dbg;
    sa.tagged = s.tagged ? 1u : 0u;
    sa.tag_limit = std::max(2u, fp.tag_limit);
    sa.taken = fp.taken;
    sa.mall_steps = fp.mall_steps;
    sa.cflags = s.cflags ? fp.cflags : nullptr;
    sa.pk_off = fp.pk_off;
    sa.pk_base = fp.pk_base;
    sa.tprof = tprof;
    return sa;
}

static AccArgs acc_args(const FastPlan &fp, const flatgfa_dev_graph_t &g, const CallShape &s, const CallHooks &hooks, uint32_t *depth_out, uint32_t *uniq_out,
                        uint32_t *status, bool psum, uint32_t *tprof) {
    AccArgs aa{};
    aa.n_segs = fp.n_range;
    aa.n_win = fp.n_win;
    aa.n_slots = fp.n_slots;
    aa.cap = fp.cap;
    aa.counts = s.kept ? fp.counts_kept : fp.counts;
    aa.counts0 = fp.counts0;
    aa.has_pre = s.has_pre2;
    aa.buckets = fp.buckets;
    aa.dir = reinterpret_cast<const uint2 *>(fp.dir);
    aa.islot = fp.islot;
    aa.dstride = fp.dstride;
    aa.elist = fp.elist;
    aa.wave_off = fp.wave_off;
    aa.n_items = fp.n_items;
    aa.work_counter = fp.work_counter;
    aa.max_back = s.max_back;
    aa.depth_out = depth_out;
    aa.uniq_out = uniq_out;
    aa.status = status;
    aa.dbg = fp.dbg;
    if (hooks.acc_skip) aa.dbg = (uint32_t)strtoul(hooks.acc_skip, nullptr, 10);
    aa.items = reinterpret_cast<const uint4 *>(fp.items);
    aa.seg_len = g.seg_len;
    aa.psum_part = psum ? reinterpret_cast<ulonglong2 *>(fp.psum_part) : nullptr;
    aa.fat_off = fp.fat_off;
    aa.fat_woff = fp.fat_woff;
    aa.parts = fp.acc_parts;
    aa.n_shared = s.tagged ? fp.n_shared : 0u;
    aa.tprof = tprof;
    aa.pair_part = fp.pair_part;
    aa.pair_flag = fp.pair_flag;
    aa.accumulate = fp.accumulate ? 1u : 0u;
    aa.taken = hooks.no_plain ? nullptr : fp.taken;
    aa.fullest = fp.taken ? fp.taken + fp.n_slots : nullptr;
    aa.pk = fp.packed ? reinterpret_cast<const uint2 *>(fp.pk) : nullptr;
    aa.keep = s.kept ? 1u : 0u;
    aa.srec = fp.sorted_rec;
    aa.scarry = fp.sorted_carry;
    aa.swin_chunk = fp.sorted_win_chunk;
    return aa;
}

static void launch_wave_lists(const FastPlan &fp, const flatgfa_dev_graph_t &g, const ScanArgs &sa, const CallShape &s, bool uniq, hipStream_t stream) {
    const struct {
        const void *items;
        uint32_t n, n_rev, mono_lo, mono_n, grid;
        int kind;
        const char *name[2];
    } lists[3] = {{fp.tiny_items, fp.n_tiny, 0u, fp.tiny_mono_lo, fp.tiny_mono_n, s.grid_tiny, 0, {"k_scan_tiny<depth>", "k_scan_tiny<uniq>"}},
                  {fp.short_items, fp.n_short, fp.n_short_rev, fp.short_mono_lo, fp.short_mono_n, s.grid_short, 1, {"k_scan_short<depth>", "k_scan_short<uniq>"}},
                  {fp.medium_items, fp.n_medium, fp.n_medium_rev, fp.medium_mono_lo, fp.medium_mono_n, s.grid_medium, 2, {"k_scan_medium<depth>", "k_scan_medium<uniq>"}}};
    for (const auto &l : lists) {
        if (!l.n) continue;
        ScanArgs sk = sa;
        sk.short_items = reinterpret_cast<const uint4 *>(l.items);
        sk.n_short = l.n;
        sk.mono_lo = l.mono_lo;
        sk.mono_n = l.mono_n;
        if (l.kind) {
            sk.n_fwd = l.n - l.n_rev;
            sk.rev_steps = fp.rev_steps;
            sk.path_begin = g.path_begin;
            sk.path_end = g.path_end;
        }
        ProfScope pscope(l.name[uniq], stream);
        if (l.kind) launch_scan_short(fp, sk, l.kind == 2, uniq, l.grid, stream);
        else launch_scan_tiny(fp, sk, uniq, l.grid, stream);
    }
}

static int run_range(const FastPlan &fp, const flatgfa_dev_graph_t &g, uint32_t *depth_out, uint32_t *uniq_out,
                     uint32_t *status, hipStream_t stream, const PathSums *ps, bool count_only, RecordsUse *records) {
    CallHooks hooks;
    hooks.scan_always = test_hook("FLATGFA_SCAN_ALWAYS") != nullptr;
    hooks.scan_time = test_hook("FLATGFA_SCAN_TIME");
    hooks.no_plain = test_hook("FLATGFA_NO_PLAIN") != nullptr;
    hooks.acc_time = test_hook("FLATGFA_ACC_TIME") != nullptr;
#ifdef FGFA_MEASURE
    hooks.acc_skip = test_hook("FLATGFA_ACC_SKIP");
#endif
    const bool uniq = uniq_out != nullptr;
    const CallShape s = decide_call(fp, {g.n_segs, g.seg_len != nullptr}, {uniq, ps != nullptr, ps && ps->clear, count_only}, hooks, records && records->use);
    if (s.refusal) { set_error(s.refusal); return FLATGFA_ERR_ARG; }
    if (records) records->from_image = s.from_image && fp.counts_kept;
    const ScanTimeDiag scan_time(hooks.scan_time, fp.n_slots);
    const AccTimeDiag acc_time(hooks.acc_time && uniq, (size_t)fp.n_win * fp.acc_parts * kAccWaves * 16);
    ScanArgs sa = scan_args(fp, g, s, status, scan_time.buf);
    AccArgs aa = acc_args(fp, g, s, hooks, depth_out, uniq_out, status, ps != nullptr, acc_time.buf);
    if (fp.n_short && hipMemsetAsync(fp.work_counter, 0, 4, stream) != hipSuccess) return FLATGFA_ERR_HIP;
    launch_wave_lists(fp, g, sa, s, uniq, stream);
    if (s.sums == Zeroes::k_scan) {
        sa.zero_c = (unsigned long long *)ps->len_out;
        sa.zero_d = (unsigned long long *)ps->weighted_out;
        sa.n_zero64 = g.n_paths;
    } else if (s.sums == Zeroes::memset) {
        ProfScope pscope("memset_path_sums", stream);
        if (hipMemsetAsync(ps->len_out, 0, (size_t)g.n_paths * 8, stream) != hipSuccess) return FLATGFA_ERR_HIP;
        if (hipMemsetAsync(ps->weighted_out, 0, (size_t)g.n_paths * 8, stream) != hipSuccess) return FLATGFA_ERR_HIP;
    }
    if (s.outputs == Zeroes::k_scan) {
        sa.zero_a = depth_out;
        sa.zero_b = uniq_out;
    } else if (s.outputs == Zeroes::memset) {
        ProfScope pscope("memset_outputs", stream);
        if (hipMemsetAsync(depth_out, 0, (size_t)fp.n_range * 4, stream) != hipSuccess) return FLATGFA_ERR_HIP;
        if (uniq_out && hipMemsetAsync(uniq_out, 0, (size_t)fp.n_range * 4, stream) != hipSuccess) return FLATGFA_ERR_HIP;
    }
    if (s.scans()) {
        ProfScope pscope(s.from_image ? "k_scan_runs" : fp.dense ? "k_scan_dense" : "k_scan", stream);
        if (s.from_image) launch_scan_runs(fp, sa, s.grid, stream);
        else if (const int rc = launch_scan(fp, sa, scan_mode(fp, s), s.grid, stream)) return rc;
    }
    if (count_only) return hipGetLastError() == hipSuccess ? FLATGFA_OK : FLATGFA_ERR_HIP;
    {
        ProfScope pscope(uniq ? "k_accum<uniq>" : (ps ? "k_accum<depth+paths>" : "k_accum<depth>"), stream);
        launch_accum(fp, aa, uniq, s.tagged, ps != nullptr, stream, s.sorted);
    }
    if (ps && fp.n_items) {
        ProfScope pscope("k_path_reduce", stream);
        launch_path_reduce(fp, (unsigned long long *)ps->len_out, (unsigned long long *)ps->weighted_out, stream);
    }
    if (hipGetLastError() != hipSuccess) {
        set_error("fast_seg_depth: kernel launch failed");
        return FLATGFA_ERR_HIP;
    }
    scan_time.report(s.grid, s.tagged, stream);
    acc_time.report(s.tagged, stream);
    if (fp.dbg & kDbgTime) report_scan_cycles(status, s.grid, stream);
    return FLATGFA_OK;
}

int fast_seg_depth(const FastPlan &fp, const flatgfa_dev_graph_t &g, uint32_t *depth_out, uint32_t *uniq_out,
                   uint32_t *status, hipStream_t stream, const PathSums *ps, RecordsUse *records) {
    if (records) records->from_image = false;
    int rc = run_range(fp, g, depth_out, uniq_out, status, stream, ps, false, records);
    for (uint32_t r = 0; r < fp.n_more && rc == FLATGFA_OK; ++r) {
        const FastPlan &q = fp.more[r];
        rc = run_range(q, g, depth_out + q.seg_base, uniq_out ? uniq_out + q.seg_base : nullptr, status, stream, nullptr, false);
    }
    return rc;
}

}
```

pollen_amd/csrc/depth_fast.hpp:

```cpp
#pragma once
#include <hip/hip_runtime_api.h>

#include <cstdint>
#include <mutex>

#include "../../include/flatgfa.h"

namespace fgfa_dev {

struct OncePerDevice {
    std::mutex mu;
    uint64_t done = 0;
    template <class F>
    bool operator()(F fn) {
        int dev = -1;
        if (hipGetDevice(&dev) != hipSuccess) return false;
        std::lock_guard<std::mutex> lk(mu);
        if (dev >= 0 && dev < 64 && ((done >> dev) & 1ull)) return true;
        if (!fn()) return false;
        if (dev >= 0 && dev < 64) done |= 1ull << dev;
        return true;
    }
};

int device_cu_count(int device);
void plan_tick(const char *what);

constexpr int kThreads = 1024;
constexpr int kWaves = kThreads / 64;
constexpr uint32_t kStBounds = 1u, kStDebug = 2u, kStOverflow = 4u, kStInternal = 8u, kStBackOverflow = 16u, kStStale = 32u;
#ifndef FGFA_MEDIUM_PAIRED
#define FGFA_MEDIUM_PAIRED 1
#endif
constexpr bool kMediumPaired = FGFA_MEDIUM_PAIRED != 0;
constexpr int kMediumHash = 11, kMediumWaves = kMediumPaired ? 14 : 8;
#ifndef FGFA_SHORT_WAVES
#define FGFA_SHORT_WAVES 16
#endif
constexpr int kShortWaves = FGFA_SHORT_WAVES;
constexpr int kModePlain = 0, kModeDbg = 1, kModeRanged = 2, kModeBig = 3, kModeRangedBig = 4, kModePacked = 5, kModePackedRanged = 6, kModePlainFlags = 7, kModePackedFlags = 8, kModePlainNarrow = 9;
constexpr bool mode_ranged(int m) { return m == kModeRanged || m == kModeRangedBig || m == kModePackedRanged; }
constexpr bool mode_big(int m) { return m == kModeBig || m == kModeRangedBig; }
constexpr bool mode_packed(int m) { return m == kModePacked || m == kModePackedRanged || m == kModePackedFlags; }
constexpr bool mode_flags(int m) { return m == kModePlainFlags || m == kModePackedFlags; }
constexpr bool mode_plain(int m) { return m == kModePlain || m == kModePlainNarrow; }
constexpr uint32_t kNoSlot = 0xFFFFFFFFu;
constexpr uint32_t kAccWaves = 16;
constexpr uint32_t kShortMax = 2048;
constexpr uint32_t kTinyMax = 128;
#ifndef FGFA_QCAP
#define FGFA_QCAP 416
#endif
constexpr uint32_t kQCap = FGFA_QCAP;
constexpr uint32_t kMediumRuns = 1500;
constexpr uint32_t kMaxHandBack = 4096;
constexpr uint32_t kTagCount = 512;
constexpr uint32_t kItemNoClaim = 0x80000000u;
constexpr uint32_t kTagSlots = 4;
constexpr uint32_t kMaxShared = 128;
constexpr uint32_t kMaxWin = 2048;
constexpr uint32_t kMaxWinTagged = 4096;

struct FastPlan {
    bool eligible = false;
    bool cap_forced = false;
    uint32_t seg_base = 0, n_range = 0;
    FastPlan *more = nullptr;
    uint32_t n_more = 0;
    uint32_t n_cus = 256;
    bool tagged = false;
    uint32_t tag_limit = 0;
    uint32_t n_shared = 0;
    bool big_groups = false;
    bool dense_maybe = false;
    bool dense = false;
    bool narrow_emit = false;
    uint32_t acc_parts = 1;
    uint64_t est_records = 0;
    bool acc_pair = false;
    uint32_t acc_slots = 4;
    bool acc_own = false;
    uint32_t *pair_part = nullptr, *pair_flag = nullptr;
    uint64_t mall_steps = 0;
    bool packed = false;
    bool can_pack = false;
    uint32_t *pk_off = nullptr;
    uint64_t *pk_base = nullptr;
    void *pk = nullptr;
    uint64_t bucket_records = 0;
    uint32_t n_slots = 0;
    uint32_t n_win = 0;
    uint32_t wb = 12;
    uint32_t nwp = 0;
    uint32_t cap = 0;
    uint32_t lds_bytes_scan = 0;
    uint32_t dbg = 0;
    uint32_t *counts = nullptr;
    uint32_t *counts0 = nullptr;
    uint32_t *buckets = nullptr;
    void *dir = nullptr;
    uint32_t *islot = nullptr;
    uint32_t *perm = nullptr;
    uint32_t dstride = 0;
    uint32_t *lists_slab = nullptr;
    uint32_t *elist = nullptr;
    uint32_t *wave_off = nullptr;
    uint32_t *fat_off = nullptr;
    uint32_t *fat_woff = nullptr;
    uint32_t n_fat = 0;
    void *items = nullptr;
    uint32_t n_items = 0;
    uint32_t n_noclaim = 0;
    uint32_t *cflags = nullptr;
    uint64_t n_flag_chunks = 0;
    bool marks_wanted = false;
    uint64_t item_steps = 0;
    uint32_t max_back = 0;
    bool accumulate = false;
    bool too_many_items = false;
    bool want_wb12 = false;
    uint32_t n_groups = 1;
    bool exact_short = false;
    void *short_items = nullptr;
    uint32_t n_short = 0, n_short_rev = 0;
    uint32_t short_mono_lo = 0, short_mono_n = 0, medium_mono_lo = 0, medium_mono_n = 0, tiny_mono_lo = 0, tiny_mono_n = 0;
    uint32_t *rev_steps = nullptr;
    uint32_t n_rev_steps = 0;
    uint32_t lds_bytes_short = 0;
    void *medium_items = nullptr;
    uint32_t n_medium = 0, n_medium_rev = 0;
    uint32_t lds_bytes_medium = 0;
    void *tiny_items = nullptr;
    uint32_t n_tiny = 0;
    uint64_t class_steps[4] = {0, 0, 0, 0};
    uint32_t lds_bytes_tiny = 0;
    uint32_t *taken = nullptr;
    uint32_t *work_counter = nullptr;
    void *psum_part = nullptr;
    uint32_t *other_ids = nullptr;
    uint32_t n_other = 0;
    const void *run_ent = nullptr;
    const void *run_item_ent = nullptr;
    uint32_t run_n_ent = 0;
    bool run_nt = false;
    uint32_t *counts_kept = nullptr;
    const uint32_t *sorted_rec = nullptr, *sorted_carry = nullptr, *sorted_win_chunk = nullptr;
    bool sorted_nt = false;
};

struct RecordsUse {
    bool use = false;
    bool from_image = false;
};

template <class Plan, class Fn>
inline void for_each_range(Plan &fp, Fn fn) {
    fn(fp);
    for (uint32_t r = 0; r < fp.n_more; ++r) {
        Plan &q = fp.more[r];
        fn(q);
    }
}
template <class Pred>
inline bool all_ranges(const FastPlan &fp, Pred pred) {
    bool all = true;
    for_each_range(fp, [&](const FastPlan &q) { all = all && pred(q); });
    return all;
}
template <class Pred>
inline bool any_range(const FastPlan &fp, Pred pred) {
    return !all_ranges(fp, [&](const FastPlan &q) { return !pred(q); });
}

struct MarksJob {
    bool active = false;
    uint32_t *vis = nullptr, *pbeg = nullptr, *chunks = nullptr, *flags = nullptr;
    unsigned long long *cnt = nullptr;
    hipEvent_t done = nullptr;
};
bool fast_marks_start(const FastPlan &fp, const flatgfa_dev_graph_t &g, const uint32_t *host_path_begin, hipStream_t side, MarksJob *job);
bool fast_marks_ready(const MarksJob &job);
void fast_marks_finish(FastPlan *fp, MarksJob *job);
int fast_check_plan_facts(const FastPlan &fp, const flatgfa_dev_graph_t &g, const uint32_t *host_path_begin, const uint32_t *host_path_end, uint32_t *status,
                          hipStream_t stream);

struct RunImage;
RunImage *run_image_start(const flatgfa_dev_graph_t &g, hipStream_t side);
int run_image_poll(RunImage *im, hipStream_t side, bool wait, uint64_t reserve, bool any_ratio);
const char *run_image_why(const RunImage *im);
uint64_t run_image_bytes(const RunImage *im);
void run_image_free(RunImage *im, hipStream_t side);
bool run_items_start(const FastPlan &fp, const RunImage *im, hipStream_t side, void **item_ent, void **room, hipEvent_t *done);
uint32_t run_room_needed(const FastPlan &fp, const void *room);
void run_image_install(FastPlan *fp, const RunImage *im, void *item_ent, bool nt);

struct SortedImage;
SortedImage *sorted_image_start(const FastPlan &fp, uint32_t n_paths, hipStream_t side);
int sorted_image_poll(SortedImage *si, const FastPlan &fp, hipStream_t side, bool wait, uint64_t reserve, bool waived);
const char *sorted_image_why(const SortedImage *si);
uint64_t sorted_image_bytes(const SortedImage *si);
uint64_t sorted_image_transient(const SortedImage *si);
int sorted_image_phase(const SortedImage *si);
void sorted_image_install(FastPlan *fp, const SortedImage *si, bool nt);
void sorted_image_free(SortedImage *si, hipStream_t side);

bool fast_plan_create(const flatgfa_dev_graph_t &g, const uint32_t *host_path_begin, const uint32_t *host_path_end,
                      FastPlan *fp, uint32_t scan_workgroups = 0, bool prefer_packed = false);
void fast_plan_destroy(FastPlan *fp);
void fast_release_scratch();
bool fast_plan_grow(FastPlan *fp, bool ahead_of_need = false);
struct PathSums {
    uint64_t *len_out, *weighted_out;
    bool clear = false;
};
bool fast_plan_want_path_sums(FastPlan *fp);
int fast_seg_depth(const FastPlan &fp, const flatgfa_dev_graph_t &g, uint32_t *depth_out, uint32_t *uniq_out,
                   uint32_t *status, hipStream_t stream, const PathSums *ps = nullptr, RecordsUse *records = nullptr);

}
```

pollen_amd/csrc/depth_fast_kernels.hpp:

```cpp
#pragma once
#include <hip/hip_runtime.h>

#include <cstdint>

#include "depth_call_host.hpp"
#include "depth_fast.hpp"
#include "device_common.hpp"

namespace fgfa_dev {


constexpr uint32_t kMaxSlots = 1024;
constexpr int kAccThreads = 1024;
static_assert(kAccThreads == 64 * (int)kAccWaves, "pass 2's workgroup is the waves the plan deals to");
constexpr uint32_t kLdsLimit = 160 * 1024;

constexpr uint32_t kRunBits = 11;
constexpr uint32_t kRunSpan = 1u << kRunBits;
constexpr uint32_t kPosBits = 10;
constexpr uint32_t kTermEntry = 0xFFFFFFFFu << kPosBits;
template <bool UNIQ>
constexpr uint32_t kCutMask = UNIQ ? 31u : kRunSpan - 1u;
constexpr uint32_t kShortWinBits = 12;
constexpr uint32_t kShortMaxWin = 256;
// ... 214 lines not shown
                   "=v"(a[8]), "=v"(a[9]), "=v"(a[10]), "=v"(a[11]), "=v"(a[12]), "=v"(a[13]), "=v"(a[14]), "=v"(a[15])  \
                 : "s"(F)                                                                                               \
                 : "memory")
template <int SET>
__device__ __forceinline__ void take_block_flagged(uint32_t (&a)[16], uint32_t f) {
    if (SET == 0) FGFA_TAKE16F(f, "v96", "v97", "v98", "v99", "v100", "v101", "v102", "v103", "v104", "v105", "v106", "v107", "v108", "v109", "v110", "v111");
    else if (SET == 2) FGFA_TAKE16F(f, "v80", "v81", "v82", "v83", "v84", "v85", "v86", "v87", "v88", "v89", "v90", "v91", "v92", "v93", "v94", "v95");
    else FGFA_TAKE16F(f, "v112", "v113", "v114", "v115", "v116", "v117", "v118", "v119", "v120", "v121", "v122", "v123", "v124", "v125", "v126", "v127");
}
template <int SET>
__device__ __forceinline__ void take_block(uint32_t (&a)[16]) {
    if (SET == 0) FGFA_TAKE16("v96", "v97", "v98", "v99", "v100", "v101", "v102", "v103", "v104", "v105", "v106", "v107", "v108", "v109", "v110", "v111");
    else if (SET == 2) FGFA_TAKE16("v80", "v81", "v82", "v83", "v84", "v85", "v86", "v87", "v88", "v89", "v90", "v91", "v92", "v93", "v94", "v95");
    else FGFA_TAKE16("v112", "v113", "v114", "v115", "v116", "v117", "v118", "v119", "v120", "v121", "v122", "v123", "v124", "v125", "v126", "v127");
}

#ifndef FGFA_SLOTS_MODE
#define FGFA_SLOTS_MODE 0
#endif
__device__ __forceinline__ uint32_t take_slots(uint32_t *bcur, int lane, bool valid, uint32_t win) {
#if FGFA_SLOTS_MODE == 1
    const unsigned long long vm = __builtin_amdgcn_ballot_w64(valid);
    if (vm == 0) return 0u;
    const uint32_t win0 = __builtin_amdgcn_readlane(win, (int)__builtin_ctzll(vm));
    if (__builtin_amdgcn_ballot_w64(valid && win != win0) == 0) {
        uint32_t first = 0;
        if (lane == 0) first = atomicAdd(&bcur[win0], (uint32_t)__builtin_popcountll(vm));
        return __builtin_amdgcn_readfirstlane(first) + lane_rank(vm);
    }
#endif
    const uint32_t key = valid ? win : 0x80000000u | (uint32_t)lane;
    const uint32_t kprev = __builtin_amdgcn_update_dpp(~0u, key, 0x138 , 0xf, 0xf, false);
    const unsigned long long heads = __builtin_amdgcn_ballot_w64(lane == 0 || key != kprev);
#if FGFA_SLOTS_MODE >= 1
    if (__builtin_popcountll(heads) > 48) return valid ? atomicAdd(&bcur[win], 1u) : 0u;
#endif
    const uint32_t head = 63u - (uint32_t)__builtin_clzll(heads & (~0ull >> (63 - lane)));
    const unsigned long long rest = (heads >> 1) >> lane;
    const uint32_t cnt = rest ? (uint32_t)__builtin_ctzll(rest) + 1u : 64u - (uint32_t)lane;
    const uint32_t first = valid && head == (uint32_t)lane ? atomicAdd(&bcur[win], cnt) : 0u;
    return (uint32_t)__builtin_amdgcn_ds_bpermute((int)(head << 2), (int)first) + ((uint32_t)lane - head);
}

constexpr uint32_t kQPacked = 64 + 944;
template <int MODE>
constexpr uint32_t kQueueOf = mode_packed(MODE) ? kQPacked : kQ2;
#ifndef FGFA_WIDE
#define FGFA_WIDE 4
#endif
constexpr int kWide = FGFA_WIDE;
constexpr int mode_wide(int m) { return m == kModePlainNarrow ? 2 : kWide; }
constexpr uint32_t kCtlRing = 32, kIdleAhead = 20;
constexpr uint32_t kCtlNext = 0, kCtlArrive = kCtlRing, kCtlEpoch = 2 * kCtlRing, kCtlJobs = 2 * kCtlRing + 8, kCtlDesc = 3 * kCtlRing + 8,
                   kCtlWords = 7 * kCtlRing + 8;
constexpr size_t kTprofRow = 4 + kWaves;
constexpr uint32_t kJobEmpty = 0xFFFFFFFFu, kJobPending = 0xFFFFFFFEu;


#ifdef __HIPCC__
__device__ __forceinline__ uint32_t wave_scan_max(uint32_t x) {
    x = max(x, (uint32_t)__builtin_amdgcn_update_dpp(0u, x, 0x111 , 0xf, 0xf, true));
    x = max(x, (uint32_t)__builtin_amdgcn_update_dpp(0u, x, 0x112 , 0xf, 0xf, true));
    x = max(x, (uint32_t)__builtin_amdgcn_update_dpp(0u, x, 0x114 , 0xf, 0xf, true));
    x = max(x, (uint32_t)__builtin_amdgcn_update_dpp(0u, x, 0x118 , 0xf, 0xf, true));
    x = max(x, (uint32_t)__builtin_amdgcn_update_dpp(0u, x, 0x142 , 0xa, 0xf, true));
    x = max(x, (uint32_t)__builtin_amdgcn_update_dpp(0u, x, 0x143 , 0xc, 0xf, true));
    return x;
}
#endif

struct AccArgs {
    uint32_t n_segs, n_win, n_slots, cap;
    uint32_t *counts;
    uint32_t *counts0;
    uint32_t has_pre;
    const uint32_t *buckets;
    const uint2 *dir;
    const uint32_t *islot;
    uint32_t dstride;
    const uint32_t *elist;
    const uint32_t *wave_off;
    uint32_t n_items;
    const uint32_t *work_counter;
    uint32_t max_back;
    uint32_t *depth_out;
    uint32_t *uniq_out;
    uint32_t *status;
    uint32_t dbg;
    const uint4 *items;
    const uint32_t *seg_len;
    ulonglong2 *psum_part;
    const uint32_t *fat_off;
    const uint32_t *fat_woff;
    uint32_t parts;
    uint32_t n_shared;
    uint32_t *tprof;
    uint32_t *pair_part;
    uint32_t *pair_flag;
    uint32_t accumulate;
    const uint32_t *taken;
    uint32_t *fullest;
    const uint2 *pk;
    uint32_t keep;
    const uint32_t *srec, *scarry, *swin_chunk;
};

struct AccTimer {
    uint32_t *buf;
    unsigned long long last;
    uint32_t acc[16];
    __device__ __forceinline__ void start(uint32_t *b) {
        buf = b;
        for (int k = 0; k < 16; ++k) acc[k] = 0;
        if (buf) last = __builtin_amdgcn_s_memrealtime();
    }
    __device__ __forceinline__ void mark(int ph) {
        if (!buf) return;
        const unsigned long long now = __builtin_amdgcn_s_memrealtime();
        acc[ph] += (uint32_t)(now - last);
        last = now;
    }
    __device__ __forceinline__ void count(int what, uint32_t n = 1u) {
        if (buf) acc[8 + what] += n;
    }
    __device__ __forceinline__ void finish() {
        if (!buf || (threadIdx.x & 63)) return;
        uint32_t *o = buf + ((size_t)(blockIdx.y * gridDim.x + blockIdx.x) * kAccWaves + (threadIdx.x >> 6)) * 16;
        for (int k = 0; k < 16; ++k) o[k] = acc[k];
    }
};

constexpr uint32_t kPCap = 96;
#ifndef FGFA_TINY_BITS
#define FGFA_TINY_BITS 8
#endif
constexpr uint32_t kTinyBits = FGFA_TINY_BITS, kTinyTab = 1u << kTinyBits;
constexpr uint32_t kTinyQueue = 64 + kTinyMax;
#ifndef FGFA_DENSE_TILE
#define FGFA_DENSE_TILE 8192
#endif
constexpr uint32_t kDenseTile = FGFA_DENSE_TILE;
constexpr int kDensePer = kDenseTile / kThreads;
inline uint32_t scan_lds_bytes(uint32_t nwp, bool tagged_only = false, bool packed = false) { return ((tagged_only && !packed ? 1u : 2u) * nwp + kCtlWords + kWaves * (packed ? kQPacked : kQ2) * 2u) * 4u; }
inline uint32_t tagged_lds_bytes(uint32_t wb, uint32_t n_shared, uint32_t slots = kTagSlots) { return (kAccWaves * slots + n_shared) * ((1u << wb) / 8u); }
inline uint32_t dense_lds_bytes(uint32_t nwp) { return (6u * nwp + 64u + kDenseTile + 64u) * 4u; }

bool scan_kernels_setup();
bool path_kernels_setup();
bool accum_kernels_setup();
int launch_scan(const FastPlan &fp, const ScanArgs &sa, ScanMode mode, uint32_t grid, hipStream_t stream);
void launch_scan_runs(const FastPlan &fp, const ScanArgs &sa, uint32_t grid, hipStream_t stream);
void launch_scan_tiny(const FastPlan &fp, const ScanArgs &sk, bool uniq, uint32_t grid, hipStream_t stream);
void launch_scan_short(const FastPlan &fp, const ScanArgs &sk, bool medium, bool uniq, uint32_t grid, hipStream_t stream);
void launch_accum(const FastPlan &fp, AccArgs &aa, bool uniq, bool tagged, bool psum, hipStream_t stream, bool sorted = false);
void launch_path_reduce(const FastPlan &fp, unsigned long long *len_out, unsigned long long *weighted_out, hipStream_t stream);

}
```

pollen_amd/csrc/depth_sorted.hip:

```cpp
#include <hip/hip_runtime.h>

#include <algorithm>
#include <vector>

#include "depth_fast_kernels.hpp"
#include "depth_sorted.hpp"
#include "depth_sorted_host.hpp"
#include "device_scan.hpp"
#include "host_copy.hpp"
#include "prof.hpp"

namespace fgfa_dev {

struct SortedImage {
    uint32_t *rec = nullptr;
    uint32_t *carry = nullptr;
    uint32_t *win_chunk = nullptr;
    uint32_t *cnt = nullptr;
    uint32_t *rec_off = nullptr;
    uint64_t *keys = nullptr;
    uint32_t *recs = nullptr;
    void *scratch = nullptr;
    uint32_t n_win = 0;
    SortedKey key;
    SortedLayout lay;
    uint64_t transient = 0;
    hipEvent_t done = nullptr;
    int phase = 0;
    const char *why = "";
};

namespace {

constexpr uint32_t kSortedHistWindows = 8192;

template <class Fn>
__device__ __forceinline__ bool sorted_records_of(const uint2 *__restrict__ ent, uint32_t i, const uint4 &d, uint32_t n_segs, uint32_t wb, Fn fn) {
    const uint32_t wmask = (1u << wb) - 1u;
    const uint2 en = ent[i];
    const uint32_t s = max(en.y, d.x), t = min(ent[i + 1u].y, d.y);
    if (s >= t) return true;
    const uint32_t skip = s - en.y, lenm1 = t - s - 1u;
    const bool dn = (en.x >> 31) != 0u;
    const uint32_t first = (en.x & 0x7FFFFFFFu) + (dn ? 0u - skip : skip);
    const uint32_t id = dn ? first - lenm1 : first;
    if (id + lenm1 >= n_segs || id + lenm1 < id) return false;
    const uint32_t win = id >> wb, rel = id & wmask;
    if (rel + lenm1 > wmask) {
        fn(win, rel, wmask - rel);
        fn(win + 1u, 0u, lenm1 - (wmask - rel) - 1u);
    } else {
        fn(win, rel, lenm1);
    }
    return true;
}

__global__ __launch_bounds__(256) void sorted_image_count(const uint4 *__restrict__ items, const uint2 *__restrict__ item_ent, uint32_t n_items,
                                                           const uint2 *__restrict__ ent, uint32_t n_segs, uint32_t wb, uint32_t n_win, uint32_t *__restrict__ cnt) {
    __shared__ uint32_t hist[kSortedHistWindows];
    const bool local = n_win <= kSortedHistWindows;
    for (uint32_t w = threadIdx.x; local && w < n_win; w += 256u) hist[w] = 0u;
    __syncthreads();
    for (uint32_t j = blockIdx.x; j < n_items; j += gridDim.x) {
        const uint4 d = items[j];
        const uint2 er = item_ent[j];
        for (uint32_t i = er.x + threadIdx.x; i < er.y; i += 256u) {
            const bool ok = sorted_records_of(ent, i, d, n_segs, wb, [&](uint32_t win, uint32_t, uint32_t) {
                if (win >= n_win) return;
                if (local) atomicAdd(&hist[win], 1u);
                else atomicAdd(&cnt[win], 1u);
            });
            if (!ok) atomicAdd(&cnt[n_win], 1u);
        }
    }
    __syncthreads();
    for (uint32_t w = threadIdx.x; local && w < n_win; w += 256u)
        if (hist[w]) atomicAdd(&cnt[w], hist[w]);
}

__global__ __launch_bounds__(256) void sorted_image_emit(const uint4 *__restrict__ items, const uint2 *__restrict__ item_ent, uint32_t n_items,
                                                          const uint2 *__restrict__ ent, uint32_t n_segs, const SortedKey key, uint32_t n_win,
                                                          uint32_t n_records, uint32_t *__restrict__ cursor, uint64_t *__restrict__ keys, uint32_t *__restrict__ recs) {
    const uint32_t wb = key.wb;
    for (uint32_t j = blockIdx.x; j < n_items; j += gridDim.x) {
        const uint4 d = items[j];
        const uint2 er = item_ent[j];
        const uint32_t path = d.w & (uint32_t)((1ull << key.path_bits) - 1ull);
        for (uint32_t i = er.x + threadIdx.x; i < er.y; i += 256u) {
            (void)sorted_records_of(ent, i, d, n_segs, wb, [&](uint32_t win, uint32_t rel, uint32_t lenm1) {
                if (win >= n_win) return;
                const uint32_t at = atomicAdd(cursor, 1u);
                if (at >= n_records) return;
                keys[at] = key.pack(win, path, rel);
                recs[at] = rel | (lenm1 << wb);
            });
        }
    }
}

__global__ __launch_bounds__(64) void sorted_image_finalise(const uint64_t *__restrict__ keys, const uint32_t *__restrict__ recs, const uint32_t *__restrict__ rec_off,
                                                            const uint32_t *__restrict__ win_chunk, uint32_t n_win, const SortedKey sk,
                                                            uint32_t *__restrict__ img, uint32_t *__restrict__ carry, uint32_t *__restrict__ wrong) {
    static_assert(kSortedChunk == 64u, "one record per lane and chunk");
    const int lane = threadIdx.x;
    const uint32_t wb = sk.wb, wmask = (1u << wb) - 1u;
    for (uint32_t w = blockIdx.x; w < n_win; w += gridDim.x) {
        const uint32_t off = rec_off[w], cnt = rec_off[w + 1u] - off, c0 = win_chunk[w], nc = win_chunk[w + 1u] - c0;
        uint32_t carry_m = 0u, carry_path = 0u;
        for (uint32_t c = 0; c < nc; ++c) {
            const uint32_t k = c * kSortedChunk + (uint32_t)lane;
            const bool have = k < cnt;
            const uint64_t key = have ? keys[off + k] : 0ull;
            const uint32_t rec = have ? recs[off + k] : 0u;
            if (have && sk.win(key) != w) atomicOr(wrong, 1u);
            const uint32_t path = sk.path(key);
            const uint32_t up = (uint32_t)__shfl_up((int)path, 1, 64);
            const uint32_t prev = lane == 0 ? carry_path : up;
            const bool first = have && (k == 0u || path != prev);
            const unsigned long long fm = __builtin_amdgcn_ballot_w64(first);
            const uint32_t ord = (uint32_t)__builtin_popcountll(fm & (~0ull >> (63 - lane)));
            const uint32_t e = (rec & wmask) + ((rec >> wb) & 1023u) + 1u;
            const uint32_t incl = wave_scan_max(have ? (ord << kSortedEndBits) | e : 0u);
            img[(size_t)(c0 + c) * kSortedChunk + lane] = have ? rec | (first ? kSortedFirst : 0u) | (ord << kSortedOrdShift) : kSortedPad;
            if (lane == 0) carry[c0 + c] = first ? 0u : carry_m;
            const uint32_t last = min(cnt - c * kSortedChunk, kSortedChunk) - 1u;
            const uint32_t incl_l = __builtin_amdgcn_readlane(incl, last), ord_l = __builtin_amdgcn_readlane(ord, last);
            const uint32_t m = incl_l & ((1u << kSortedEndBits) - 1u);
            carry_m = ord_l == 0u ? max(carry_m, m) : m;
            carry_path = __builtin_amdgcn_readlane(path, last);
        }
    }
}

void sorted_release_scratch(SortedImage *si) {
    for (void **p : {(void **)&si->cnt, (void **)&si->rec_off, (void **)&si->keys, (void **)&si->recs, &si->scratch}) {
        if (*p) (void)hipFree(*p);
        *p = nullptr;
    }
}

int sorted_fail(SortedImage *si, const char *why) {
    (void)hipGetLastError();
    sorted_release_scratch(si);
    for (void **p : {(void **)&si->rec, (void **)&si->carry, (void **)&si->win_chunk}) {
        if (*p) (void)hipFree(*p);
        *p = nullptr;
    }
    si->phase = -1;
    si->why = why;
    return -1;
}

}

SortedImage *sorted_image_start(const FastPlan &fp, uint32_t n_paths, hipStream_t side) {
    auto *si = new SortedImage();
    si->n_win = fp.n_win;
    si->key = sorted_key(fp.wb, n_paths, fp.n_win);
    if (!fp.run_ent || !fp.run_item_ent || !fp.n_items || !fp.n_win) {
        sorted_fail(si, "error");
        return si;
    }
    if (si->key.bits() > 64) {
        sorted_fail(si, "size");
        return si;
    }
    const size_t cnt_bytes = ((size_t)fp.n_win + 3) * 4;
    if (hipMalloc(&si->cnt, cnt_bytes) != hipSuccess || hipEventCreateWithFlags(&si->done, hipEventDisableTiming) != hipSuccess) {
        sorted_fail(si, "memory");
        return si;
    }
    {
        ProfScope ps("sorted_image_count", side);
        if (hipMemsetAsync(si->cnt, 0, cnt_bytes, side) != hipSuccess) {
            sorted_fail(si, "error");
            return si;
        }
        hipLaunchKernelGGL(sorted_image_count, dim3(std::min<uint32_t>(fp.n_items, fp.n_cus * 8u)), dim3(256), 0, side, reinterpret_cast<const uint4 *>(fp.items),
                           reinterpret_cast<const uint2 *>(fp.run_item_ent), fp.n_items, reinterpret_cast<const uint2 *>(fp.run_ent), fp.n_range, fp.wb, fp.n_win, si->cnt);
    }
    if (hipEventRecord(si->done, side) != hipSuccess || hipGetLastError() != hipSuccess) {
        (void)hipStreamSynchronize(side);
        sorted_fail(si, "error");
        return si;
    }
    si->phase = 1;
    return si;
}

int sorted_image_poll(SortedImage *si, const FastPlan &fp, hipStream_t side, bool wait, uint64_t reserve, bool waived) {
    for (;;) {
        if (si->phase == 3) return 1;
        if (si->phase < 1) return -1;
        if (wait) {
            if (hipEventSynchronize(si->done) != hipSuccess) return sorted_fail(si, "error");
        } else if (hipEventQuery(si->done) != hipSuccess) {
            (void)hipGetLastError();
            return 0;
        }
        if (si->phase == 2) {
            uint32_t end[2] = {0u, 1u};
            if (staged_copy(end, si->cnt + si->n_win + 1, 8, hipMemcpyDeviceToHost, nullptr) != hipSuccess) return sorted_fail(si, "error");
            if (end[0] != si->lay.n_records || end[1]) return sorted_fail(si, "stale");
            sorted_release_scratch(si);
            si->phase = 3;
            return 1;
        }
        std::vector<uint32_t> cnt((size_t)si->n_win + 1);
        if (staged_copy(cnt.data(), si->cnt, cnt.size() * 4, hipMemcpyDeviceToHost, nullptr) != hipSuccess) return sorted_fail(si, "error");
        if (cnt[si->n_win]) return sorted_fail(si, "bounds");
        si->lay = sorted_layout(cnt.data(), si->n_win);
        if (!si->lay.fits || !si->lay.n_records) return sorted_fail(si, "size");
        const uint32_t n = (uint32_t)si->lay.n_records;
        size_t scratch_bytes = 0;
        if (!sorted_sort_pairs(nullptr, &scratch_bytes, nullptr, nullptr, nullptr, nullptr, n, side)) return sorted_fail(si, "error");
        si->transient = sorted_transient_bytes(n, si->n_win, scratch_bytes);
        const uint64_t kept = sorted_kept_bytes(si->lay.n_chunks, si->n_win);
        size_t free_b = 0, total_b = 0;
        if (hipMemGetInfo(&free_b, &total_b) != hipSuccess) {
            (void)hipGetLastError();
            free_b = 0;
        }
        if (sorted_memory_refused(si->transient, kept, free_b, reserve, waived)) return sorted_fail(si, "memory");
        if (hipMalloc(&si->keys, (size_t)n * 16) != hipSuccess || hipMalloc(&si->recs, (size_t)n * 8) != hipSuccess ||
            hipMalloc(&si->scratch, std::max<size_t>(scratch_bytes, 16)) != hipSuccess || hipMalloc(&si->rec_off, ((size_t)si->n_win + 1) * 4) != hipSuccess ||
            hipMalloc(&si->rec, si->lay.n_chunks * kSortedChunk * 4) != hipSuccess || hipMalloc(&si->carry, si->lay.n_chunks * 4) != hipSuccess ||
            hipMalloc(&si->win_chunk, ((size_t)si->n_win + 1) * 4) != hipSuccess)
            return sorted_fail(si, "memory");
        if (staged_copy(si->rec_off, si->lay.rec_off.data(), ((size_t)si->n_win + 1) * 4, hipMemcpyHostToDevice, side) != hipSuccess ||
            staged_copy(si->win_chunk, si->lay.win_chunk.data(), ((size_t)si->n_win + 1) * 4, hipMemcpyHostToDevice, side) != hipSuccess)
            return sorted_fail(si, "error");
        const uint4 *items = reinterpret_cast<const uint4 *>(fp.items);
        {
            ProfScope ps("sorted_image_emit", side);
            hipLaunchKernelGGL(sorted_image_emit, dim3(std::min<uint32_t>(fp.n_items, fp.n_cus * 8u)), dim3(256), 0, side, items, reinterpret_cast<const uint2 *>(fp.run_item_ent),
                               fp.n_items, reinterpret_cast<const uint2 *>(fp.run_ent), fp.n_range, si->key, fp.n_win, n, si->cnt + si->n_win + 1, si->keys, si->recs);
        }
        {
            ProfScope ps("sorted_image_sort", side);
            if (!sorted_sort_pairs(si->scratch, &scratch_bytes, si->keys, si->keys + n, si->recs, si->recs + n, n, side)) {
                (void)hipStreamSynchronize(side);
                return sorted_fail(si, "error");
            }
        }
        {
            ProfScope ps("sorted_image_finalise", side);
            hipLaunchKernelGGL(sorted_image_finalise, dim3(fp.n_win), dim3(64), 0, side, si->keys + n, si->recs + n, si->rec_off, si->win_chunk, fp.n_win, si->key,
                               si->rec, si->carry, si->cnt + si->n_win + 2);
        }
        if (hipEventRecord(si->done, side) != hipSuccess || hipGetLastError() != hipSuccess) {
            (void)hipStreamSynchronize(side);
            return sorted_fail(si, "error");
        }
        si->phase = 2;
    }
}

const char *sorted_image_why(const SortedImage *si) { return si->why; }
int sorted_image_phase(const SortedImage *si) { return si->phase; }
uint64_t sorted_image_bytes(const SortedImage *si) { return si->phase == 3 ? sorted_kept_bytes(si->lay.n_chunks, si->n_win) : 0; }
uint64_t sorted_image_transient(const SortedImage *si) { return si->transient; }

void sorted_image_install(FastPlan *fp, const SortedImage *si, bool nt) {
    fp->sorted_rec = si->rec;
    fp->sorted_carry = si->carry;
    fp->sorted_win_chunk = si->win_chunk;
    fp->sorted_nt = nt;
}

void sorted_image_free(SortedImage *si, hipStream_t side) {
    if (!si) return;
    if (si->phase == 1 || si->phase == 2) (void)hipStreamSynchronize(side);
    sorted_release_scratch(si);
    for (void *p : {(void *)si->rec, (void *)si->carry, (void *)si->win_chunk})
        if (p) (void)hipFree(p);
    if (si->done) (void)hipEventDestroy(si->done);
    delete si;
}

}
```

pollen_amd/csrc/depth_sorted_host.hpp:

```cpp
#pragma once
#include <algorithm>
#include <cstdint>
#include <vector>

#ifdef __HIPCC__
#define FGFA_SORTED_HD __host__ __device__
#else
#define FGFA_SORTED_HD
#endif

namespace fgfa_dev {

constexpr uint32_t kSortedK = 1;
constexpr uint32_t kSortedChunk = 64u * kSortedK;
constexpr uint32_t kSortedFirst = 1u << 23;
constexpr uint32_t kSortedPad = 1u << 31;
constexpr uint32_t kSortedEndBits = 14;
constexpr uint32_t kSortedOrdShift = 24;
constexpr uint32_t kSortedOrdMask = 0x7Fu;
constexpr uint32_t kSortedGroup = 4;
constexpr uint32_t kSortedQShift = kSortedEndBits + 7;
static_assert(kSortedOrdShift + 7 == 31 && kSortedQShift + 2 <= 24, "the ordinal lies between the first-of-path flag and the padding flag; the key fits a word");

inline uint32_t bits_for(uint64_t n_values) {
    uint32_t b = 0;
    while (b < 64 && (n_values - 1) >> b && n_values > 1) ++b;
    return b;
}

struct SortedKey {
    uint32_t wb = 0, path_bits = 0, win_bits = 0;
    FGFA_SORTED_HD uint32_t bits() const { return wb + path_bits + win_bits; }
    FGFA_SORTED_HD uint64_t pack(uint32_t win, uint32_t path, uint32_t rel) const { return ((((uint64_t)win << path_bits) | path) << wb) | rel; }
    FGFA_SORTED_HD uint32_t path(uint64_t key) const { return (uint32_t)((key >> wb) & ((1ull << path_bits) - 1ull)); }
    FGFA_SORTED_HD uint32_t win(uint64_t key) const { return (uint32_t)(key >> (wb + path_bits)); }
    FGFA_SORTED_HD uint32_t rel(uint64_t key) const { return (uint32_t)(key & ((1ull << wb) - 1ull)); }
};
inline SortedKey sorted_key(uint32_t wb, uint32_t n_paths, uint32_t n_win) {
    SortedKey k;
    k.wb = wb;
    k.path_bits = std::max(1u, bits_for(n_paths));
    k.win_bits = std::max(1u, bits_for(n_win));
    return k;
}

struct SortedLayout {
    std::vector<uint32_t> rec_off;
    std::vector<uint32_t> win_chunk;
    uint64_t n_records = 0, n_chunks = 0;
    bool fits = true;
};
inline SortedLayout sorted_layout(const uint32_t *win_count, uint32_t n_win) {
    SortedLayout l;
    l.rec_off.resize((size_t)n_win + 1);
    l.win_chunk.resize((size_t)n_win + 1);
    for (uint32_t w = 0; w < n_win; ++w) {
        l.rec_off[w] = (uint32_t)l.n_records;
        l.win_chunk[w] = (uint32_t)l.n_chunks;
        l.n_records += win_count[w];
        l.n_chunks += ((uint64_t)win_count[w] + kSortedChunk - 1) / kSortedChunk;
        if (l.n_records >= (1ull << 31) || l.n_chunks * kSortedChunk >= (1ull << 31)) l.fits = false;
    }
    l.rec_off[n_win] = (uint32_t)l.n_records;
    l.win_chunk[n_win] = (uint32_t)l.n_chunks;
    return l;
}

inline uint64_t sorted_kept_bytes(uint64_t n_chunks, uint32_t n_win) { return n_chunks * kSortedChunk * 4 + n_chunks * 4 + ((uint64_t)n_win + 1) * 4; }
inline uint64_t sorted_transient_bytes(uint64_t n_records, uint32_t n_win, uint64_t sort_scratch) {
    return n_records * (8 + 4) * 2 + sort_scratch + ((uint64_t)n_win + 1) * 4 + 16;
}
inline bool sorted_memory_refused(uint64_t transient, uint64_t kept, uint64_t free_bytes, uint64_t reserve, bool waived) {
    return !waived && transient + kept + reserve > free_bytes;
}

inline const char *sorted_refused(int hook, uint32_t acc_parts, uint32_t n_groups, uint32_t n_more, uint32_t wb, bool keeps_records) {
    if (hook == 0) return "hook";
    if (!keeps_records) return "rewritten";
    if (acc_parts != 1) return "parts";
    if (n_groups > 1 || n_more) return "ranges";
    if (wb < 11 || wb > 13) return "windows";
    return nullptr;
}

FGFA_SORTED_HD inline uint32_t sorted_umax(uint32_t a, uint32_t b) { return a > b ? a : b; }
FGFA_SORTED_HD inline uint32_t sorted_umin(uint32_t a, uint32_t b) { return a < b ? a : b; }
FGFA_SORTED_HD inline uint32_t sorted_seed(uint32_t q, uint32_t carry) { return (q << kSortedQShift) | carry; }

struct SortedLane {
    uint32_t s[kSortedGroup], len[kSortedGroup], x[kSortedGroup];
    uint32_t t;
};
template <bool CHECKED>
FGFA_SORTED_HD inline void sorted_lane_keys(const uint32_t (&rec)[kSortedGroup], uint32_t q, uint32_t wb, uint32_t seed, SortedLane &ln) {
    ln.t = seed;
    for (uint32_t k = 0; k < kSortedGroup; ++k) {
        ln.s[k] = rec[k] & ((1u << wb) - 1u);
        ln.len[k] = (rec[k] >> wb) & 1023u;
        const uint32_t x = ((rec[k] >> (kSortedOrdShift - kSortedEndBits)) & (kSortedOrdMask << kSortedEndBits)) | ((q << kSortedQShift) + ln.s[k] + ln.len[k] + 1u);
        ln.x[k] = CHECKED && (rec[k] & kSortedPad) ? 0u : x;
        ln.t = sorted_umax(ln.t, ln.x[k]);
    }
}
template <bool CHECKED>
FGFA_SORTED_HD inline bool sorted_record_step(uint32_t &p, uint32_t x, uint32_t len, uint32_t &end) {
    const bool hit = (!CHECKED || x != 0u) && p >= x - len;
    end = sorted_umin(x, p) & ((1u << kSortedEndBits) - 1u);
    p = sorted_umax(p, x);
    return hit;
}

}
```

Measured before the change: 11710 billion.

## Pack depth and revisit deltas into one LDS word for sorted accumulation

Adds a packed cell mode to the sorted accumulation kernel that holds the depth and revisit difference counters in one 32-bit LDS word (16 bits each). The number of atomics per record drops from up to four to two or three, and LDS use is halved. A preprocessing kernel computes per-window maximum start and end counts so packing is only chosen when the values fit in 16 bits. It also adds an optional 'solo' mode that requests half the CU's LDS per workgroup to limit co-residency, but that mode is off by default.

After: 11970 billion (median of 6 runs). 2.2% higher.

```diff
diff --git a/pollen_amd/csrc/depth_accum.hip b/pollen_amd/csrc/depth_accum.hip
--- a/pollen_amd/csrc/depth_accum.hip
+++ b/pollen_amd/csrc/depth_accum.hip
@@ -2,6 +2,9 @@
 
 #include <cstdlib>
 
+#include <algorithm>
+
+#include "depth_call_host.hpp"
 #include "depth_fast_kernels.hpp"
 #include "depth_sorted_host.hpp"
 
@@ -217,6 +220,22 @@
         block_scan<int, kPer>(reinterpret_cast<int *>(wave_tot), v);
 #pragma unroll
         for (int k = 0; k < kPer; ++k) d[k] = (uint32_t)v[k];
+    }
+}
+template <int kPer>
+__device__ __forceinline__ void window_counts_packed(const uint32_t *W, unsigned long long *wave_tot, uint32_t i0, uint32_t (&d)[kPer], uint32_t (&rv)[kPer]) {
+    unsigned long long v[kPer];
+#pragma unroll
+    for (int k = 0; k < kPer; ++k) {
+        int32_t dd, dr;
+        sorted_unpack(W[i0 + k], dd, dr);
+        v[k] = (unsigned long long)(long long)dd + ((unsigned long long)(long long)dr << 32);
+    }
+    block_scan<unsigned long long, kPer>(wave_tot, v);
+#pragma unroll
+    for (int k = 0; k < kPer; ++k) {
+        d[k] = (uint32_t)v[k];
+        rv[k] = (uint32_t)(v[k] >> 32);
     }
 }
 template <bool UNIQ, int kPer>
@@ -1149,7 +1168,7 @@
 template <bool NT>
 __device__ __forceinline__ sorted_u32x4 sorted_load4(const sorted_u32x4 *p) { return NT ? __builtin_nontemporal_load(p) : *p; }
 
-template <bool UNIQ, int WB, bool CHECKED>
+template <bool UNIQ, int WB, bool CHECKED, bool PACKED>
 __device__ __forceinline__ void sweep_group(int *D, int *R, const sorted_u32x4 &r4, uint32_t carry, bool in, int lane) {
     const uint32_t pad = CHECKED && !in ? kSortedPad : 0u;
     const uint32_t rec[kSortedGroup] = {r4.x | pad, r4.y | pad, r4.z | pad, r4.w | pad};
@@ -1158,6 +1177,13 @@
         SortedLane ln;
         sorted_lane_keys<CHECKED>(rec, q, (uint32_t)WB, seed, ln);
         uint32_t p = sorted_umax(seed, wave_scan_max((uint32_t)__builtin_amdgcn_update_dpp(0u, ln.t, 0x138 , 0xf, 0xf, true)));
+        if (PACKED) {
+            uint32_t *W = reinterpret_cast<uint32_t *>(D);
+#pragma unroll
+            for (uint32_t k = 0; k < kSortedGroup; ++k)
+                sorted_record_packed<CHECKED>(p, ln.s[k], ln.len[k], ln.x[k], [&](uint32_t cell, uint32_t v) { atomicAdd(&W[cell], v); });
+            return;
+        }
 #pragma unroll
         for (uint32_t k = 0; k < kSortedGroup; ++k) {
             uint32_t end;
@@ -1184,14 +1210,16 @@
     }
 }
 
-template <bool UNIQ, int WB, bool NT>
+template <bool UNIQ, int WB, bool NT, bool PACKED = false>
 __global__ __launch_bounds__(kAccThreads) __attribute__((amdgpu_waves_per_eu(8, 8))) void k_accum_sorted(const AccArgs A) {
+    static_assert(UNIQ || !PACKED, "packed cells hold depth and revisits: the depth-only builds have one array as it is");
     static_assert(kSortedChunk == 64u && kSortedGroup == 4u, "a lane holds four consecutive records of one chunk: sixteen lanes a chunk");
     constexpr uint32_t kW = 1u << WB;
     constexpr int kPer = kW / kAccThreads;
-    __shared__ __attribute__((aligned(16))) int cells[(UNIQ ? 2 : 1) * (kW + 64)];
+    constexpr uint32_t kCells = (UNIQ && !PACKED ? 2u : 1u) * (kW + 64);
+    __shared__ __attribute__((aligned(16))) int cells[kCells];
     __shared__ unsigned long long wave_tot[kAccWaves];
-    int *D = cells, *R = cells + (UNIQ ? kW + 64 : 0);
+    int *D = cells, *R = cells + (UNIQ && !PACKED ? kW + 64 : 0);
     const int tid = threadIdx.x, lane = tid & 63;
     const uint32_t wave = __builtin_amdgcn_readfirstlane(tid >> 6);
     const uint32_t win = blockIdx.x, w0 = win * kW;
@@ -1208,11 +1236,11 @@
         if (UNIQ) cy = A.scarry[min(ck + q, c1 - 1u)];
     };
     const auto sweep = [&](const sorted_u32x4 &r, uint32_t cy, uint32_t at) {
-        if (at + 1u == ng) sweep_group<UNIQ, WB, true>(D, R, r, cy, c0 + at * kSortedGroup + q < c1, lane);
-        else sweep_group<UNIQ, WB, false>(D, R, r, cy, true, lane);
+        if (at + 1u == ng) sweep_group<UNIQ, WB, true, PACKED>(D, R, r, cy, c0 + at * kSortedGroup + q < c1, lane);
+        else sweep_group<UNIQ, WB, false, PACKED>(D, R, r, cy, true, lane);
     };
     if (ng) request(ra, ca, g);
-    for (uint32_t i = tid; i < (UNIQ ? 2u : 1u) * (kW + 64); i += kAccThreads) cells[i] = 0;
+    for (uint32_t i = tid; i < kCells; i += kAccThreads) cells[i] = 0;
     __syncthreads();
     while (g < ng) {
         request(rb, cb, g + kAccWaves);
@@ -1226,7 +1254,8 @@
     __syncthreads();
     const uint32_t nvalid = min(kW, A.n_segs - w0), i0 = kPer * tid;
     uint32_t d[kPer], u[kPer];
-    window_counts<UNIQ, kPer>(D, R, wave_tot, i0, d, u);
+    if (PACKED) window_counts_packed<kPer>(reinterpret_cast<const uint32_t *>(D), wave_tot, i0, d, u);
+    else window_counts<UNIQ, kPer>(D, R, wave_tot, i0, d, u);
     if (UNIQ) {
 #pragma unroll
         for (int k = 0; k < kPer; ++k) u[k] = d[k] - u[k];
@@ -1234,6 +1263,15 @@
     write_counts<UNIQ, kPer>(A, w0, i0, nvalid, A.accumulate != 0u, d, u);
 }
 
+}
+
+uint32_t device_cu_lds_bytes() {
+    int dev = 0, per_cu = 0, per_wg = 0;
+    if (hipGetDevice(&dev) != hipSuccess) return 0u;
+    if (hipDeviceGetAttribute(&per_cu, hipDeviceAttributeMaxSharedMemoryPerMultiprocessor, dev) != hipSuccess) per_cu = 0;
+    if (hipDeviceGetAttribute(&per_wg, hipDeviceAttributeMaxSharedMemoryPerBlock, dev) != hipSuccess) per_wg = 0;
+    (void)hipGetLastError();
+    return (uint32_t)std::max(0, std::max(per_cu, per_wg));
 }
 
 bool accum_kernels_setup() {
@@ -1259,6 +1297,17 @@
         set((const void *)k_accum<true, 12, false, false, false, true, (int)kTagSlots, true, true>, tagged_lds_bytes(12, kMaxShared));
         set((const void *)k_accum<true, 12, false, false, false, true, 8, true, true>, tagged_lds_bytes(12, 64, 8));
         set((const void *)k_accum<true, 13, false, false, false, true, (int)kTagSlots, true, true>, tagged_lds_bytes(13, 0));
+        const uint32_t solo = sorted_solo_lds(1, 2u, device_cu_lds_bytes());
+#define FGFA_SORTED_SET(WB_)                                                                                                    \
+        set((const void *)k_accum_sorted<true, WB_, false, true>, solo), set((const void *)k_accum_sorted<true, WB_, true, true>, solo),   \
+        set((const void *)k_accum_sorted<true, WB_, false>, solo), set((const void *)k_accum_sorted<true, WB_, true>, solo),               \
+        set((const void *)k_accum_sorted<false, WB_, false>, solo), set((const void *)k_accum_sorted<false, WB_, true>, solo)
+        if (solo) {
+            FGFA_SORTED_SET(11);
+            FGFA_SORTED_SET(12);
+            FGFA_SORTED_SET(13);
+        }
+#undef FGFA_SORTED_SET
 #ifdef FGFA_MEASURE
         set((const void *)k_accum_small<11>, tagged_lds_bytes(11, kMaxShared));
         set((const void *)k_accum_pair<12, false>, tagged_lds_bytes(12, 0));
@@ -1282,13 +1331,16 @@
     } while (0)
 #define FGFA_SORTED_LAUNCH(WB_)                                                                                                  \
     do {                                                                                                                        \
-        if (uniq && fp.sorted_nt) hipLaunchKernelGGL((k_accum_sorted<true, WB_, true>), dim3(fp.n_win), dim3(kAccThreads), 0, stream, aa);        \
-        else if (uniq) hipLaunchKernelGGL((k_accum_sorted<true, WB_, false>), dim3(fp.n_win), dim3(kAccThreads), 0, stream, aa);                  \
-        else if (fp.sorted_nt) hipLaunchKernelGGL((k_accum_sorted<false, WB_, true>), dim3(fp.n_win), dim3(kAccThreads), 0, stream, aa);          \
-        else hipLaunchKernelGGL((k_accum_sorted<false, WB_, false>), dim3(fp.n_win), dim3(kAccThreads), 0, stream, aa);                           \
+        if (uniq && packed && fp.sorted_nt) hipLaunchKernelGGL((k_accum_sorted<true, WB_, true, true>), dim3(fp.n_win), dim3(kAccThreads), sorted_lds, stream, aa);  \
+        else if (uniq && packed) hipLaunchKernelGGL((k_accum_sorted<true, WB_, false, true>), dim3(fp.n_win), dim3(kAccThreads), sorted_lds, stream, aa);            \
+        else if (uniq && fp.sorted_nt) hipLaunchKernelGGL((k_accum_sorted<true, WB_, true>), dim3(fp.n_win), dim3(kAccThreads), sorted_lds, stream, aa);   \
+        else if (uniq) hipLaunchKernelGGL((k_accum_sorted<true, WB_, false>), dim3(fp.n_win), dim3(kAccThreads), sorted_lds, stream, aa);                  \
+        else if (fp.sorted_nt) hipLaunchKernelGGL((k_accum_sorted<false, WB_, true>), dim3(fp.n_win), dim3(kAccThreads), sorted_lds, stream, aa);          \
+        else hipLaunchKernelGGL((k_accum_sorted<false, WB_, false>), dim3(fp.n_win), dim3(kAccThreads), sorted_lds, stream, aa);                           \
     } while (0)
-void launch_accum(const FastPlan &fp, AccArgs &aa, bool uniq, bool tagged, bool psum, hipStream_t stream, bool sorted) {
+void launch_accum(const FastPlan &fp, AccArgs &aa, bool uniq, bool tagged, bool psum, hipStream_t stream, bool sorted, uint32_t sorted_lds) {
     if (sorted) {
+        const bool packed = fp.sorted_cells == kSortedCellsPacked;
         if (fp.wb == 11) FGFA_SORTED_LAUNCH(11);
         else if (fp.wb == 12) FGFA_SORTED_LAUNCH(12);
         else FGFA_SORTED_LAUNCH(13);
diff --git a/pollen_amd/csrc/depth_call_host.hpp b/pollen_amd/csrc/depth_call_host.hpp
--- a/pollen_amd/csrc/depth_call_host.hpp
+++ b/pollen_amd/csrc/depth_call_host.hpp
@@ -33,6 +33,7 @@
     bool from_image = false;
     bool kept = false;
     bool sorted = false;
+    uint32_t sorted_solo_lds = 0;
     uint32_t has_pre2 = 0;
     uint32_t max_back = 0;
     Zeroes outputs = Zeroes::nobody, sums = Zeroes::nobody;
@@ -58,6 +59,10 @@
     if (s.ranged) return {kModeRanged, s.tagged};
     return {s.tagged && fp.narrow_emit ? kModePlainNarrow : kModePlain, s.tagged};
 }
+
+constexpr bool kSortedLanesSoloDefault = false;
+inline bool sorted_lanes_solo(int hook, uint32_t lanes) { return hook >= 0 ? hook == 1 : kSortedLanesSoloDefault && lanes >= 2u; }
+inline uint32_t sorted_solo_lds(int hook, uint32_t lanes, uint32_t cu_lds_bytes) { return sorted_lanes_solo(hook, lanes) ? cu_lds_bytes / 2u : 0u; }
 
 inline uint32_t wave_list_grid(uint32_t n, uint32_t per_wg, uint32_t n_slots) { return std::min<uint32_t>((n + per_wg - 1) / per_wg, n_slots); }
 
@@ -85,6 +90,7 @@
     s.from_image = s.grid && tagged && fp.run_ent && fp.run_item_ent && !w.count_only && !fp.dense && !fp.packed && !s.ranged && !s.cflags && !s.has_pre && !fp.dbg;
     s.kept = s.from_image && records_use && fp.counts_kept;
     s.sorted = s.kept && fp.sorted_rec && fp.sorted_carry && fp.sorted_win_chunk && fp.acc_parts == 1 && fp.wb >= 11 && fp.wb <= 13;
+    s.sorted_solo_lds = s.sorted ? fp.sorted_solo_lds : 0u;
     if (s.scans() && !s.from_image && scan_mode(fp, s).mode == kModeRefused) {
         CallShape no;
         no.refusal = "fast_seg_depth: a bucket array this large needs a tagged call";
diff --git a/pollen_amd/csrc/depth_device.hip b/pollen_amd/csrc/depth_device.hip
--- a/pollen_amd/csrc/depth_device.hip
+++ b/pollen_amd/csrc/depth_device.hip
@@ -267,6 +267,8 @@
     int sorted_state = 0;
     const char *sorted_off = "";
     int sorted_hook = -1;
+    uint32_t lanes = 0;
+    bool sorted_said = false;
 };
 
 static int plan_fast_call(flatgfa_dev_plan_t *pl, uint32_t *depth_out, uint32_t *uniq_out, hipStream_t stream, const PathSums *ps = nullptr) {
@@ -574,6 +576,10 @@
     }
 }
 
+static void sorted_lanes_apply(flatgfa_dev_plan_t *pl) {
+    const char *hook = test_hook("FLATGFA_SORTED_SOLO");
+    pl->fast.sorted_solo_lds = sorted_solo_lds(!hook ? -1 : !strcmp(hook, "1") ? 1 : !strcmp(hook, "0") ? 0 : -1, pl->lanes, device_cu_lds_bytes());
+}
 static void sorted_poll(flatgfa_dev_plan_t *pl, bool wait) {
     if (pl->sorted_state == 3 || pl->sorted_state < 0 || pl->run_state != 3) return;
     const auto give_up = [&](const char *why) {
@@ -613,6 +619,8 @@
     const char *mall = getenv("FLATGFA_MALL_MB");
     const bool nt = traffic > (244ll << 20) || (mall && strtoull(mall, nullptr, 10) == 0);
     sorted_image_install(&pl->fast, pl->sorted->img, nt);
+    sorted_lanes_apply(pl);
+    pl->sorted_said = test_hook("FLATGFA_SORTED_CELLS") || test_hook("FLATGFA_SORTED_SOLO");
     pl->sorted_state = 3;
 }
 
@@ -1243,6 +1251,8 @@
                     s += std::string(" pass2=walk(") + (pl->sorted_state < 0 ? pl->sorted_off : "pending") + ")";
                 }
                 s += std::string(" records=") + (pl->keep_records && f.counts_kept ? "kept" : "rewritten");
+                if (pl->sorted_state == 3 && f.sorted_rec && pl->sorted_said)
+                    s += std::string(" sorted_cells=") + sorted_cells_name(f.sorted_cells) + " sorted_lanes=" + (f.sorted_solo_lds ? "solo" : "shared");
             } else {
                 s += std::string(" run_image=off(") + (pl->run_state < 0 ? pl->run_off : "pending") + ")";
             }
@@ -1357,6 +1367,8 @@
         const uint32_t wgs = calls_in_flight < 2 ? 0u : (uint32_t)(calls_in_flight >= 3 && g->n_steps <= (1ull << 28) ? n_cus / 2 : n_cus * 11 / 16);
         flatgfa_dev_plan_t *pl = plan_create_impl(g, hb, he, wgs);
         if (!pl) { flatgfa_dev_pipeline_destroy(p); return nullptr; }
+        pl->lanes = (uint32_t)calls_in_flight;
+        if (pl->sorted_state == 3) sorted_lanes_apply(pl);
         p->plans.push_back(pl);
     }
     if (hipEventCreateWithFlags(&p->after, hipEventDisableTiming) != hipSuccess) { set_error("dev_pipeline_create: cannot create an event"); flatgfa_dev_pipeline_destroy(p); return nullptr; }
diff --git a/pollen_amd/csrc/depth_fast.hip b/pollen_amd/csrc/depth_fast.hip
--- a/pollen_amd/csrc/depth_fast.hip
+++ b/pollen_amd/csrc/depth_fast.hip
@@ -1352,7 +1352,7 @@
     if (count_only) return hipGetLastError() == hipSuccess ? FLATGFA_OK : FLATGFA_ERR_HIP;
     {
         ProfScope pscope(uniq ? "k_accum<uniq>" : (ps ? "k_accum<depth+paths>" : "k_accum<depth>"), stream);
-        launch_accum(fp, aa, uniq, s.tagged, ps != nullptr, stream, s.sorted);
+        launch_accum(fp, aa, uniq, s.tagged, ps != nullptr, stream, s.sorted, s.sorted_solo_lds);
     }
     if (ps && fp.n_items) {
         ProfScope pscope("k_path_reduce", stream);
diff --git a/pollen_amd/csrc/depth_fast.hpp b/pollen_amd/csrc/depth_fast.hpp
--- a/pollen_amd/csrc/depth_fast.hpp
+++ b/pollen_amd/csrc/depth_fast.hpp
@@ -24,6 +24,7 @@
 };
 
 int device_cu_count(int device);
+uint32_t device_cu_lds_bytes();
 void plan_tick(const char *what);
 
 constexpr int kThreads = 1024;
@@ -146,6 +147,8 @@
     uint32_t *counts_kept = nullptr;
     const uint32_t *sorted_rec = nullptr, *sorted_carry = nullptr, *sorted_win_chunk = nullptr;
     bool sorted_nt = false;
+    uint32_t sorted_cells = 0;
+    uint32_t sorted_solo_lds = 0;
 };
 
 struct RecordsUse {
diff --git a/pollen_amd/csrc/depth_fast_kernels.hpp b/pollen_amd/csrc/depth_fast_kernels.hpp
--- a/pollen_amd/csrc/depth_fast_kernels.hpp
+++ b/pollen_amd/csrc/depth_fast_kernels.hpp
@@ -390,7 +390,7 @@
 void launch_scan_runs(const FastPlan &fp, const ScanArgs &sa, uint32_t grid, hipStream_t stream);
 void launch_scan_tiny(const FastPlan &fp, const ScanArgs &sk, bool uniq, uint32_t grid, hipStream_t stream);
 void launch_scan_short(const FastPlan &fp, const ScanArgs &sk, bool medium, bool uniq, uint32_t grid, hipStream_t stream);
-void launch_accum(const FastPlan &fp, AccArgs &aa, bool uniq, bool tagged, bool psum, hipStream_t stream, bool sorted = false);
+void launch_accum(const FastPlan &fp, AccArgs &aa, bool uniq, bool tagged, bool psum, hipStream_t stream, bool sorted = false, uint32_t sorted_lds = 0);
 void launch_path_reduce(const FastPlan &fp, unsigned long long *len_out, unsigned long long *weighted_out, hipStream_t stream);
 
 }
diff --git a/pollen_amd/csrc/depth_sorted.hip b/pollen_amd/csrc/depth_sorted.hip
--- a/pollen_amd/csrc/depth_sorted.hip
+++ b/pollen_amd/csrc/depth_sorted.hip
@@ -1,6 +1,8 @@
 #include <hip/hip_runtime.h>
 
 #include <algorithm>
+#include <cstdlib>
+#include <cstring>
 #include <vector>
 
 #include "depth_fast_kernels.hpp"
@@ -25,6 +27,7 @@
     SortedKey key;
     SortedLayout lay;
     uint64_t transient = 0;
+    uint32_t cell_max[2] = {0u, 0u};
     hipEvent_t done = nullptr;
     int phase = 0;
     const char *why = "";
@@ -132,6 +135,31 @@
     }
 }
 
+constexpr uint32_t kSortedMaxWb = 13;
+__global__ __launch_bounds__(256) void sorted_image_cell_max(const uint32_t *__restrict__ img, const uint32_t *__restrict__ win_chunk, uint32_t wb, uint32_t *__restrict__ out) {
+    __shared__ uint32_t hist[(1u << kSortedMaxWb) + 1u];
+    __shared__ uint32_t top;
+    const uint32_t w = blockIdx.x, wmask = (1u << wb) - 1u, n_cells = (1u << wb) + 1u;
+    const uint32_t r0 = win_chunk[w] * kSortedChunk, r1 = win_chunk[w + 1u] * kSortedChunk;
+    for (uint32_t pass = 0; pass < 2u; ++pass) {
+        for (uint32_t i = threadIdx.x; i < n_cells; i += 256u) hist[i] = 0u;
+        if (threadIdx.x == 0) top = 0u;
+        __syncthreads();
+        for (uint32_t i = r0 + threadIdx.x; i < r1; i += 256u) {
+            const uint32_t rec = img[i];
+            const uint32_t s = rec & wmask, cell = pass ? s + ((rec >> wb) & 1023u) + 1u : s;
+            if (!(rec & kSortedPad) && cell < n_cells) atomicAdd(&hist[cell], 1u);
+        }
+        __syncthreads();
+        uint32_t m = 0u;
+        for (uint32_t i = threadIdx.x; i < n_cells; i += 256u) m = max(m, hist[i]);
+        if (m) atomicMax(&top, m);
+        __syncthreads();
+        if (threadIdx.x == 0 && top) atomicMax(&out[pass], top);
+        __syncthreads();
+    }
+}
+
 void sorted_release_scratch(SortedImage *si) {
     for (void **p : {(void **)&si->cnt, (void **)&si->rec_off, (void **)&si->keys, (void **)&si->recs, &si->scratch}) {
         if (*p) (void)hipFree(*p);
@@ -165,7 +193,7 @@
         sorted_fail(si, "size");
         return si;
     }
-    const size_t cnt_bytes = ((size_t)fp.n_win + 3) * 4;
+    const size_t cnt_bytes = ((size_t)fp.n_win + 5) * 4;
     if (hipMalloc(&si->cnt, cnt_bytes) != hipSuccess || hipEventCreateWithFlags(&si->done, hipEventDisableTiming) != hipSuccess) {
         sorted_fail(si, "memory");
         return si;
@@ -199,9 +227,11 @@
             return 0;
         }
         if (si->phase == 2) {
-            uint32_t end[2] = {0u, 1u};
-            if (staged_copy(end, si->cnt + si->n_win + 1, 8, hipMemcpyDeviceToHost, nullptr) != hipSuccess) return sorted_fail(si, "error");
+            uint32_t end[4] = {0u, 1u, 0u, 0u};
+            if (staged_copy(end, si->cnt + si->n_win + 1, 16, hipMemcpyDeviceToHost, nullptr) != hipSuccess) return sorted_fail(si, "error");
             if (end[0] != si->lay.n_records || end[1]) return sorted_fail(si, "stale");
+            si->cell_max[0] = end[2];
+            si->cell_max[1] = end[3];
             sorted_release_scratch(si);
             si->phase = 3;
             return 1;
@@ -248,6 +278,10 @@
             hipLaunchKernelGGL(sorted_image_finalise, dim3(fp.n_win), dim3(64), 0, side, si->keys + n, si->recs + n, si->rec_off, si->win_chunk, fp.n_win, si->key,
                                si->rec, si->carry, si->cnt + si->n_win + 2);
         }
+        if (fp.wb <= kSortedMaxWb) {
+            ProfScope ps("sorted_image_cell_max", side);
+            hipLaunchKernelGGL(sorted_image_cell_max, dim3(fp.n_win), dim3(256), 0, side, si->rec, si->win_chunk, fp.wb, si->cnt + si->n_win + 3);
+        }
         if (hipEventRecord(si->done, side) != hipSuccess || hipGetLastError() != hipSuccess) {
             (void)hipStreamSynchronize(side);
             return sorted_fail(si, "error");
@@ -266,6 +300,9 @@
     fp->sorted_carry = si->carry;
     fp->sorted_win_chunk = si->win_chunk;
     fp->sorted_nt = nt;
+    const char *hook = std::getenv("FLATGFA_SORTED_CELLS");
+    const int forced = !hook ? -1 : !strcmp(hook, "packed") ? 1 : !strcmp(hook, "wide") ? 0 : -1;
+    fp->sorted_cells = sorted_cells_choice(forced, si->cell_max[0], si->cell_max[1]);
 }
 
 void sorted_image_free(SortedImage *si, hipStream_t side) {
diff --git a/pollen_amd/csrc/depth_sorted_host.hpp b/pollen_amd/csrc/depth_sorted_host.hpp
--- a/pollen_amd/csrc/depth_sorted_host.hpp
+++ b/pollen_amd/csrc/depth_sorted_host.hpp
@@ -110,4 +110,34 @@
     return hit;
 }
 
+constexpr uint32_t kSortedPackRevisit = 1u << 16;
+constexpr uint32_t kSortedPackLimit = 1u << 14;
+FGFA_SORTED_HD inline uint32_t sorted_pack(int32_t dD, int32_t dR) { return (uint32_t)dD + ((uint32_t)dR << 16); }
+FGFA_SORTED_HD inline void sorted_unpack(uint32_t w, int32_t &dD, int32_t &dR) {
+    dD = (int32_t)(int16_t)(uint16_t)(w & 0xFFFFu);
+    dR = (int32_t)(int16_t)(uint16_t)((w - (uint32_t)dD) >> 16);
 }
+FGFA_SORTED_HD inline uint32_t sorted_pack_start(bool hit) { return 1u + (hit ? kSortedPackRevisit : 0u); }
+FGFA_SORTED_HD inline uint32_t sorted_pack_end(bool hit_to_e) { return 1u + (hit_to_e ? kSortedPackRevisit : 0u); }
+template <bool CHECKED, class Add>
+FGFA_SORTED_HD inline void sorted_record_packed(uint32_t &p, uint32_t s, uint32_t len, uint32_t x, Add add) {
+    uint32_t end;
+    const bool hit = sorted_record_step<CHECKED>(p, x, len, end);
+    if (CHECKED && x == 0u) return;
+    const uint32_t e = s + len + 1u;
+    add(s, sorted_pack_start(hit));
+    add(e, 0u - sorted_pack_end(hit && end == e));
+    if (hit && end != e) add(end, 0u - kSortedPackRevisit);
+}
+inline bool sorted_cells_fit(uint32_t max_starts, uint32_t max_ends) { return max_starts != 0u && max_starts < kSortedPackLimit && max_ends < kSortedPackLimit; }
+constexpr uint32_t kSortedCellsUnknown = 0, kSortedCellsPacked = 1, kSortedCellsWideRule = 2, kSortedCellsWideHook = 3;
+inline uint32_t sorted_cells_choice(int hook, uint32_t max_starts, uint32_t max_ends) {
+    if (max_starts == 0u) return kSortedCellsUnknown;
+    if (!sorted_cells_fit(max_starts, max_ends)) return kSortedCellsWideRule;
+    return hook == 0 ? kSortedCellsWideHook : kSortedCellsPacked;
+}
+inline const char *sorted_cells_name(uint32_t cells) {
+    return cells == kSortedCellsPacked ? "packed" : cells == kSortedCellsWideRule ? "wide(rule)" : cells == kSortedCellsWideHook ? "wide(hook)" : "wide(unknown)";
+}
+
+}
```
